# LargeWorldModel/LWM

Measured on AMD Instinct MI355X. Metric: tokens/sec fwd+bwd, LWM-7B RingAttention hot path (32 layers x 32 heads x 128), higher is better.
Workload: dtype bf16 (f32 logits/softmax/accumulate)

## Files before the change

lwm_amd/csrc/attn_bwd64.h:

```cpp
#pragma once

namespace lwm {

constexpr int kD4BK = 128;
constexpr int kD4BQ = 64;
constexpr int kD4Threads = 256;
constexpr int kD4Slots = 4;
constexpr int kD4TileBytes = kD4BQ * kRowBytes;
constexpr int kD4SlotBytes = 2 * kD4TileBytes;
constexpr int kD4OffStat = kD4Slots * kD4SlotBytes;
constexpr int kD4StatBytes = 3 * kD4BQ * 4;
constexpr int kD4LdsBytes = kD4OffStat + kD4Slots * kD4StatBytes;
#ifndef LWM_D4_AHEAD
#define LWM_D4_AHEAD 6
#endif
constexpr int kD4Ahead = LWM_D4_AHEAD;
static_assert(kD4Ahead >= 1 && kD4Ahead <= 7, "prefetch distance in fragments");
static_assert((kD4Ahead % 2) == 0, "paired requests need an even distance");

struct D4Ctx {
    uint32_t qa[8];
    uint32_t tlo[4], tup[4];
    uint32_t plo[4], pup[4];
    uint32_t stat;
    float c;
    int hi;
};

#ifdef LWM_EMU
LWM_DEVICE void d4_mfma_p_first(f32x16& d, bf16x8 a, bf16x8 b) { d = mfma_32x32x16(a, b, d); }
LWM_DEVICE void d4_mfma_o_first(f32x16& d, bf16x8 a, bf16x8 b) { d = mfma_32x32x16(a, b, zero_f32x16()); }
LWM_DEVICE float d4_mul(float a, float b) { return a * b; }
LWM_DEVICE void d4_dma_b32(uint32_t voff, const char* src, lds_t dst) { glds_load_b32(src + voff, dst); }
LWM_DEVICE void d4_settle_t(f32x16&) {}
LWM_DEVICE void d4_settle_acc(f32x16 (&)[4], f32x16 (&)[4]) {}
LWM_DEVICE void d4_settle_acc4(f32x16 (&)[4]) {}
#else
LWM_DEVICE void d4_mfma_p_first(f32x16& d, bf16x8 a, bf16x8 b) {
    asm volatile("s_nop 1\n\tv_mfma_f32_32x32x16_bf16 %0, %1, %2, %0" : "+v"(d) : "v"(a), "a"(b));
}
LWM_DEVICE void d4_mfma_o_first(f32x16& d, bf16x8 a, bf16x8 b) {
    asm volatile("v_mfma_f32_32x32x16_bf16 %0, %1, %2, 0" : "=&a"(d) : "v"(a), "v"(b));
}
LWM_DEVICE float d4_mul(float a, float b) {
    float y;
    asm volatile("v_mul_f32 %0, %1, %2" : "=v"(y) : "v"(a), "v"(b));
    return y;
}
LWM_DEVICE void d4_dma_b32(uint32_t voff, const char* src, lds_t dst) {
    const uint64_t a = (uint64_t)src;
    const uint64_t u = ((uint64_t)(uint32_t)__builtin_amdgcn_readfirstlane((int)(a >> 32)) << 32) |
                       (uint32_t)__builtin_amdgcn_readfirstlane((int)a);
    asm volatile("s_mov_b32 m0, %2\n\ts_nop 0\n\tglobal_load_lds_dword %0, %1" ::"v"(voff), "s"(u), "s"(dst) : "memory");
}
LWM_DEVICE void d4_settle_t(f32x16& s) { asm volatile("s_nop 7\n\ts_nop 7" : "+v"(s)); }
LWM_DEVICE void d4_settle_acc(f32x16 (&a)[4], f32x16 (&b)[4]) {
    asm volatile("s_nop 7\n\ts_nop 7"
                 : "+a"(a[0]), "+a"(a[1]), "+a"(a[2]), "+a"(a[3]), "+a"(b[0]), "+a"(b[1]), "+a"(b[2]), "+a"(b[3]));
}
LWM_DEVICE void d4_settle_acc4(f32x16 (&a)[4]) { asm volatile("s_nop 7\n\ts_nop 7" : "+a"(a[0]), "+a"(a[1]), "+a"(a[2]), "+a"(a[3])); }
#endif

LWM_DEVICE void d4_stage_offsets(const AttnParams& p, int wave, int lane, int st, uint32_t (&vq)[4], uint32_t (&vdo)[4]) {
    const int slot = lane & 15;
    for (int j = 0; j < 4; ++j) {
        const int row = 4 * (wave + 4 * j) + (lane >> 4);
        int qrow = st * kD4BQ + row;
        qrow = qrow < p.Sq ? qrow : p.Sq - 1;
        const int rel = qrow - st * kD4BQ;
        const int col = (slot ^ swz(row)) << 3;
        vq[j] = (uint32_t)(((int64_t)rel * p.q_ss + col) * 2);
        vdo[j] = (uint32_t)(((int64_t)rel * p.do_ss + col) * 2);
    }
}

template <int HALF>
LWM_DEVICE bf16x8 d4_frag(const D4Ctx& cx, int f) {
    if (f >= 32) {
        const int g = f - 32;
        return lds_read_b128(cx.qa[g >> 1] + (g & 1) * kD4TileBytes + (HALF == 0 ? 32 * kRowBytes : 0));
    }
    if (f < 16) return lds_read_b128(cx.qa[f >> 1] + (f & 1) * kD4TileBytes + HALF * 32 * kRowBytes);
    const int j = f - 16, t = (j >> 3) & 1, db = (j >> 1) & 3;
    const uint32_t alo = HALF == 0 ? cx.plo[db] : cx.tlo[db];
    const uint32_t aup = HALF == 0 ? cx.pup[db] : cx.tup[db];
    const uint32_t off = ((j & 1) ? 0 : kD4TileBytes) + (HALF == 0 ? 32 * kRowBytes : 0) + 16 * t * kRowBytes;
    bf16x4 lo = lds_read_tr16(alo + off);
    bf16x4 up = lds_read_tr16(aup + off);
    bf16x8 o;
    o[0] = lo[0]; o[1] = lo[1]; o[2] = lo[2]; o[3] = lo[3];
    o[4] = up[0]; o[5] = up[1]; o[6] = up[2]; o[7] = up[3];
    return o;
}

struct D4Sched {
    int F[16], E[16], M[16], P[8], D[8];
};
constexpr bool d4_sched_ok(const D4Sched& c) {
    for (int e = 0; e < 16; ++e) {
        if (c.F[e] < 1 || c.F[e] > 15) return false;
        if (c.E[e] <= c.F[e] || c.M[e] <= c.E[e] || c.M[e] > 29) return false;
    }
    for (int i = 0; i < 8; ++i) {
        const int lo = i < 4 ? 8 : 16;
        if (c.P[i] < lo || c.P[i] > 29 || c.P[i] <= c.E[2 * i] || c.P[i] <= c.E[2 * i + 1]) return false;
        if (c.D[i] < lo || c.D[i] > 29 || c.D[i] <= c.M[2 * i] || c.D[i] <= c.M[2 * i + 1]) return false;
    }
    return true;
}
constexpr D4Sched kD4Sched = {
     {1, 1, 2, 2, 3, 3, 4, 4, 5, 5, 6, 6, 7, 7, 8, 8},
     {2, 3, 4, 4, 5, 6, 7, 7, 8, 9, 9, 10, 10, 11, 11, 12},
     {16, 16, 17, 17, 18, 18, 19, 19, 20, 20, 21, 21, 22, 22, 23, 23},
     {16, 17, 18, 19, 20, 21, 22, 23},
     {24, 25, 26, 27, 28, 29, 29, 29}};
static_assert(d4_sched_ok(kD4Sched), "filler schedule violates a dependency");

struct D4Dma {
    const char* q_src;
    const char* do_src;
    lds_t dst;
};

struct D4Regs {
    f32x16 s;
    f32x16 dp[2];
    float nl[16];
    float t[16];
    float ds[16];
    bf16x8 pb[2], dsb[2];
    uint32_t pw[8], dw[8];
    bf16x8 fr[8];
};

template <int G>
LWM_DEVICE void d4_fillers(const D4Ctx& cx, D4Regs& rg, const f32x16& dpu) {
#pragma unroll
    for (int e = 0; e < 16; ++e) {
        if (kD4Sched.F[e] == G) rg.t[e] = f4_fma(rg.s[e], cx.c, rg.nl[e]);
        if (kD4Sched.E[e] == G) rg.t[e] = f4_exp2(rg.t[e]);
        if (kD4Sched.M[e] == G) rg.ds[e] = d4_mul(rg.t[e], dpu[e]);
    }
#pragma unroll
    for (int i = 0; i < 8; ++i) {
        if (kD4Sched.P[i] == G) rg.pw[i] = f4_cvt_pk(rg.t[2 * i], rg.t[2 * i + 1]);
        if (kD4Sched.D[i] == G) rg.dw[i] = f4_cvt_pk(rg.ds[2 * i], rg.ds[2 * i + 1]);
    }
#pragma unroll
    for (int h = 0; h < 2; ++h) {
        int lp = 0, ld = 0;
        for (int i = 4 * h; i < 4 * h + 4; ++i) {
            lp = kD4Sched.P[i] > lp ? kD4Sched.P[i] : lp;
            ld = kD4Sched.D[i] > ld ? kD4Sched.D[i] : ld;
        }
        if (lp == G) rg.pb[h] = __builtin_bit_cast(bf16x8, u32x4{rg.pw[4 * h], rg.pw[4 * h + 1], rg.pw[4 * h + 2], rg.pw[4 * h + 3]});
        if (ld == G) rg.dsb[h] = __builtin_bit_cast(bf16x8, u32x4{rg.dw[4 * h], rg.dw[4 * h + 1], rg.dw[4 * h + 2], rg.dw[4 * h + 3]});
    }
}
template <int G0, int N>
LWM_DEVICE void d4_fill_at(int g, const D4Ctx& cx, D4Regs& rg, const f32x16& dpu) {
    if constexpr (N > 0) {
        if (g == G0) d4_fillers<G0>(cx, rg, dpu);
        else d4_fill_at<G0 + 1, N - 1>(g, cx, rg, dpu);
    }
}

template <int HALF>
LWM_DEVICE void d4_load_ndelta(uint32_t stat, f32x16& dp, int g) {
    const f32x4 v = lds_read_f32x4(stat + kD4BQ * 4 + HALF * 32 * 4 + 8 * g * 4);
    dp[4 * g + 0] = v[0]; dp[4 * g + 1] = v[1]; dp[4 * g + 2] = v[2]; dp[4 * g + 3] = v[3];
}

template <int HALF, bool HAS_PREV, bool DMA>
LWM_DEVICE void d4_x(const D4Ctx& cx, D4Regs& rg, const bf16x8 (&kf)[8], const bf16x8 (&vf)[8], const uint32_t (&vq)[4],
                     const uint32_t (&vdo)[4], const D4Dma& dm) {
    f32x16& dpn = rg.dp[HALF];
    const f32x16& dpo = rg.dp[HALF ^ 1];
#pragma unroll
    for (int m = 0; m < 16; ++m) {
        if ((m & 1) == 0) {
            rg.fr[(m + kD4Ahead) & 7] = d4_frag<HALF>(cx, m + kD4Ahead);
            rg.fr[(m + kD4Ahead + 1) & 7] = d4_frag<HALF>(cx, m + kD4Ahead + 1);
        }
        if ((m & 3) == 2) {
            const int g = m >> 2;
            const f32x4 v = lds_read_f32x4(cx.stat + HALF * 32 * 4 + 8 * g * 4);
            rg.nl[4 * g + 0] = v[0]; rg.nl[4 * g + 1] = v[1]; rg.nl[4 * g + 2] = v[2]; rg.nl[4 * g + 3] = v[3];
        }
        sched_fence();
        {
            const int f = m ^ 1;
            if (f == 0) f4_mfma_s_first(rg.s, rg.fr[0], kf[0]);
            else if ((f & 1) == 0) f4_mfma_s(rg.s, rg.fr[f & 7], kf[f >> 1]);
            else if (f == 1) d4_mfma_p_first(dpn, rg.fr[1], vf[0]);
            else f4_mfma_s(dpn, rg.fr[f & 7], vf[f >> 1]);
        }
        if (DMA && (m & 1)) {
            const int j = m >> 2;
            if ((m & 2) == 0) f4_dma1(vq[j], dm.q_src, dm.dst + 4096 * j);
            else f4_dma1(vdo[j], dm.do_src, dm.dst + kD4TileBytes + 4096 * j);
        }
        if (HAS_PREV) d4_fill_at<16, 16>(16 + m, cx, rg, dpo);
        sched_fence();
    }
}

template <int HALF, bool HAS_META>
LWM_DEVICE void d4_mask(const D4Ctx& cx, D4Regs& rg, int rel, int32_t kseg) {
#pragma unroll
    for (int g = 0; g < 4; ++g) {
        if (HAS_META) {
            const u32x4 sg = lds_read_u32x4(cx.stat + 2 * kD4BQ * 4 + HALF * 32 * 4 + 8 * g * 4);
#pragma unroll
            for (int j = 0; j < 4; ++j) {
                const bool vis = ((int32_t)sg[j] == kseg) && (8 * g + j >= rel);
                rg.s[4 * g + j] = vis ? rg.s[4 * g + j] : -INFINITY;
            }
        } else {
#pragma unroll
            for (int j = 0; j < 4; ++j) rg.s[4 * g + j] = (8 * g + j >= rel) ? rg.s[4 * g + j] : -INFINITY;
        }
    }
}

template <int HALF, bool HAS_PREV, bool NEXT, bool INIT>
LWM_DEVICE void d4_y(const D4Ctx& cx, D4Regs& rg, f32x16 (&dk)[4], f32x16 (&dv)[4], uint32_t statn) {
#pragma unroll
    for (int j = 0; j < 16; ++j) {
        const int m = 16 + j;
        if ((j & 1) == 0 && (m + kD4Ahead < 32 || NEXT)) {
            rg.fr[(m + kD4Ahead) & 7] = d4_frag<HALF>(cx, m + kD4Ahead);
            rg.fr[(m + kD4Ahead + 1) & 7] = d4_frag<HALF>(cx, m + kD4Ahead + 1);
        }
        if (NEXT && j >= 12) d4_load_ndelta<HALF ^ 1>(statn, rg.dp[HALF ^ 1], j - 12);
        sched_fence();
        if (HAS_PREV) {
            const int jf = j ^ 1;
            if (INIT && jf < 8) {
                if ((jf & 1) == 0) d4_mfma_o_first(dv[(jf >> 1) & 3], rg.fr[(16 + jf) & 7], rg.pb[0]);
                else d4_mfma_o_first(dk[(jf >> 1) & 3], rg.fr[(16 + jf) & 7], rg.dsb[0]);
            } else {
                if ((jf & 1) == 0) f4_mfma_o(dv[(jf >> 1) & 3], rg.fr[(16 + jf) & 7], rg.pb[jf >> 3]);
                else f4_mfma_o(dk[(jf >> 1) & 3], rg.fr[(16 + jf) & 7], rg.dsb[jf >> 3]);
            }
        }
        d4_fill_at<0, 16>(j, cx, rg, rg.dp[HALF]);
        sched_fence();
    }
}

template <int PAR>
LWM_DEVICE void d4_drain(const D4Ctx& cx, D4Regs& rg, f32x16 (&dk)[4], f32x16 (&dv)[4]) {
#pragma unroll
    for (int g = 16; g < 32; ++g) d4_fill_at<16, 16>(g, cx, rg, rg.dp[PAR]);
#pragma unroll
    for (int h = 0; h < 2; ++h) {
#pragma unroll
        for (int j = 0; j < 8; ++j) rg.fr[j] = d4_frag<0>(cx, 16 + 8 * h + j);
        sched_fence();
#pragma unroll
        for (int j = 0; j < 8; ++j) {
            const int jj = 8 * h + j;
            if ((jj & 1) == 0) f4_mfma_o(dv[(jj >> 1) & 3], rg.fr[j], rg.pb[jj >> 3]);
            else f4_mfma_o(dk[(jj >> 1) & 3], rg.fr[j], rg.dsb[jj >> 3]);
        }
        sched_fence();
    }
}

LWM_DEVICE void d4_store_tiles(const AttnParams& p, lds_t tb, const f32x16 (&dk)[4], const f32x16 (&dv)[4], int b, int h,
                               int row0, int lane) {
    const int l31 = lane & 31, hi = lane >> 5, col = l31 * 4;
    const int Sk = p.Sk;
    const bool carry = p.carry_in != 0, fin = p.final_out != 0;
    const int rows = Sk - (row0 + hi);
    const int64_t acc0 = ((((int64_t)b * Sk + row0 + hi) * p.H + h) * kHeadDim + col) * 4;
    const int64_t acc_step = (int64_t)2 * p.H * kHeadDim * 4;
#pragma unroll
    for (int which = 0; which < 2; ++which) {
        if (which) wave_lds_fence();
        epi_tile_write(tb, which ? dv : dk, which ? 1.0f : p.scale, l31, hi);
        wave_lds_fence();
        char* ap = (char*)(which ? p.dv_acc : p.dk_acc) + acc0;
        const int64_t o_ss = which ? p.dv_ss : p.dk_ss;
        char* op = (char*)((which ? p.dv : p.dk) + (int64_t)b * (which ? p.dv_sb : p.dk_sb) + (int64_t)(row0 + hi) * o_ss +
                           (int64_t)h * (which ? p.dv_sh : p.dk_sh) + col);
        const int64_t out_step = 2 * o_ss * 2;
        if (fin && !carry) {
#pragma unroll
            for (int i = 0; i < 16; ++i) {
                const f32x4 x = epi_tile_read(tb, i, lane);
                if (2 * i < rows) global_store_b64(op + i * out_step, u32x2{pack_bf16x2(x[0], x[1]), pack_bf16x2(x[2], x[3])});
            }
        } else if (!fin && !carry) {
#pragma unroll
            for (int i = 0; i < 16; ++i) {
                const f32x4 x = epi_tile_read(tb, i, lane);
                if (2 * i < rows) global_store_f32x4((float*)(ap + i * acc_step), x);
            }
        } else {
#pragma unroll
            for (int i = 0; i < 16; ++i) {
                f32x4 x = epi_tile_read(tb, i, lane);
                if (2 * i < rows) {
                    const f32x4 c = global_load_f32x4((const float*)(ap + i * acc_step));
                    x[0] += c[0]; x[1] += c[1]; x[2] += c[2]; x[3] += c[3];
                    if (fin) global_store_b64(op + i * out_step, u32x2{pack_bf16x2(x[0], x[1]), pack_bf16x2(x[2], x[3])});
                    else global_store_f32x4((float*)(ap + i * acc_step), x);
                }
            }
        }
    }
}

template <bool HAS_META>
LWM_DEVICE void attn_bwd_dkdv4_body(const AttnParams& p) {
#ifdef LWM_PROF
    const unsigned long long d4_entry = __builtin_amdgcn_s_memtime();
    unsigned long long d4_head = 0, d4_epi = 0;
#endif
    const lds_t lds = dyn_lds();
    const int tid = thread_idx();
    const int wave = wave_uniform(tid >> 6), lane = tid & 63, l31 = lane & 31, hi = lane >> 5;

    const int nkb = (p.Sk + kD4BK - 1) / kD4BK;
    const int HB = p.H * p.B;
    int lin = block_idx_x(), kbi, hb;
    if ((HB & 7) == 0) {
        int xcd = lin & 7, i = lin >> 3;
        hb = xcd + 8 * (i / nkb);
        kbi = i % nkb;
    } else {
        hb = lin / nkb;
        kbi = lin % nkb;
    }
    const int b = hb / p.H, h = hb % p.H;
    const bf16_t* qb = p.q + (int64_t)b * p.q_sb + (int64_t)h * p.q_sh;
    const bf16_t* kb = p.k + (int64_t)b * p.k_sb + (int64_t)h * p.k_sh;
    const bf16_t* vb = p.v + (int64_t)b * p.v_sb + (int64_t)h * p.v_sh;
    const bf16_t* dob = p.dout + (int64_t)b * p.do_sb + (int64_t)h * p.do_sh;

    const int k_row = kbi * kD4BK + wave * 32 + l31;
    const bool k_ok = k_row < p.Sk;
    const int kr = k_ok ? k_row : p.Sk - 1;
    bf16x8 kf[8], vf[8];
    for (int s = 0; s < 8; ++s) kf[s] = f4_load_agpr(kb + (int64_t)kr * p.k_ss + 16 * s + 8 * hi);
    for (int s = 0; s < 8; ++s) vf[s] = f4_load_agpr(vb + (int64_t)kr * p.v_ss + 16 * s + 8 * hi);
    const PosMap qm = q_map(p);
    const PosTab qt_ = load_postab(qm);
    const int64_t k_base = pos_base(load_postab(k_map(p)), kbi * kD4BK);
    const int64_t k_pos = k_base + k_row;
    int32_t kseg = 0;
    if (HAS_META) {
        kseg = kSegInvalid;
        if (k_ok) {
            const bool valid = p.key_valid ? (p.key_valid[(int64_t)b * p.Sk + k_row] != 0) : true;
            if (valid) kseg = p.seg_k ? p.seg_k[(int64_t)b * p.Sk + k_row] : 0;
        }
    }

    int nst = (p.Sq + kD4BQ - 1) / kD4BQ;
    int st0 = 0;
    if (p.causal) st0 = tiles_below(qt_, kD4BQ, nst, k_base + (int64_t)kbi * kD4BK - 1);
    if (HAS_META && p.segb_q && p.segb_k && st0 < nst) {
        const int nbq = (p.Sq + 31) >> 5, nbk = (p.Sk + 31) >> 5;
        int smin, smax, lo, hi2;
        seg_own_range(p.segb_k + (int64_t)b * nbk * 2, nbk, kbi * (kD4BK / 32), kD4BK / 32, smin, smax);
        seg_narrow<kD4Threads>(p.segb_q + (int64_t)b * nbq * 2, nbq, kD4BQ / 32, st0, nst, smin, smax, lds + kD4OffStat, tid, lo, hi2);
        st0 = lo;
        nst = hi2;
    }
    const int n = nst > st0 ? nst - st0 : 0;

    f32x16 dk[4], dv[4];
    if (n == 0)
        for (int i = 0; i < 4; ++i) {
            dk[i] = zero_f32x16();
            dv[i] = zero_f32x16();
        }
    if (n == 0) {
        f4_load_agpr_wait8(kf);
        f4_load_agpr_wait8(vf);
    }

    if (n > 0) {
        D4Ctx cx;
        cx.hi = hi;
        cx.c = p.scale * kLog2e;
        for (int s = 0; s < 8; ++s) cx.qa[s] = lds + tile_off(l31, 2 * s + hi);
        {
            const TrFragAddr t = frag_tr_addr(lds, lane);
            for (int db = 0; db < 4; ++db) {
                cx.tlo[db] = t.lo[db];
                cx.tup[db] = t.up[db];
                cx.plo[db] = t.lo[db];
                cx.pup[db] = t.up[db];
            }
        }
        cx.stat = lds + kD4OffStat + 16 * hi;

        const int64_t q_step_bytes = (int64_t)kD4BQ * p.q_ss * 2, do_step_bytes = (int64_t)kD4BQ * p.do_ss * 2;
        uint32_t vq[4], vdo[4];
        d4_stage_offsets(p, wave, lane, 0, vq, vdo);
        const int64_t Sqp = bwd_stat_pad(p.Sq);
        const char* stat_src = (const char*)(p.delta + bwd_stat_row((int64_t)b * p.H + h, Sqp) + (wave == 1 ? Sqp : 0));
        bool stat_on = wave < 2;
        if (HAS_META && wave == 2 && p.seg_q) {
            stat_src = (const char*)(p.seg_q + (int64_t)b * p.Sq);
            stat_on = true;
        }
        const lds_t stat_dst = lds + kD4OffStat + (uint32_t)(wave < 3 ? wave : 0) * kD4BQ * 4;
        const uint32_t vstat = (uint32_t)lane * 4;
        if (HAS_META && !p.seg_q)
            for (int sl = 0; sl < kD4Slots; ++sl)
                if (tid < kD4BQ) lds_write_i32(lds + kD4OffStat + sl * kD4StatBytes + 2 * kD4BQ * 4 + tid * 4, 0);
        auto stage_step = [&](int i) {
            const int st = nst - 1 - i;
            const lds_t dst = lds + (i & 3) * kD4SlotBytes + (uint32_t)wave * 1024;
            const char* qs = (const char*)qb + st * q_step_bytes;
            const char* ds = (const char*)dob + st * do_step_bytes;
            if (stat_on) {
                int row = st * kD4BQ + lane;
                if (HAS_META && wave == 2) row = row < p.Sq ? row : p.Sq - 1;
                glds_load_b32(stat_src + (int64_t)row * 4, stat_dst + (i & 3) * kD4StatBytes);
            }
            if (st * kD4BQ + kD4BQ > p.Sq) {
                uint32_t v2[4], d2[4];
                d4_stage_offsets(p, wave, lane, st, v2, d2);
                f4_dma<4>(v2, qs, dst);
                f4_dma<4>(d2, ds, dst + kD4TileBytes);
            } else {
                f4_dma<4>(vq, qs, dst);
                f4_dma<4>(vdo, ds, dst + kD4TileBytes);
            }
        };

        stage_step(0);
        if (n > 1) stage_step(1);
        f4_load_agpr_wait8(kf);
        f4_load_agpr_wait8(vf);
        block_sync();

        auto clamp32 = [](int64_t x) -> int { return x > (1 << 30) ? (1 << 30) : (x < -(1 << 30) ? -(1 << 30) : (int)x); };
        const int k_rel = clamp32(k_pos - p.q_start) - 4 * hi;
        PosCursor qc = cursor_begin(qt_);
        auto q_rel_of = [&](int ub) -> int {
            cursor_seek(qm, qc, ub);
            return clamp32(qc.base + ub - p.q_start);
        };
        const int mask_end = p.causal ? 32 * tiles_reaching(qt_, 32, (p.Sq + 31) / 32, k_base + (int64_t)kbi * kD4BK + wave * 32 + 31 - 1) : 0;
        auto needs_causal = [&](int ub) -> bool { return ub < mask_end; };
        const int32_t own_seg = wave_uniform(kseg);
        const bool own_uniform = HAS_META && !wave_any(kseg != own_seg || kseg == kSegInvalid);
        auto rel_of = [&](int ub) -> int {
            if (!p.causal) return -64;
            const int64_t d = (int64_t)k_rel - q_rel_of(ub);
            return d > 64 ? 64 : (d < -64 ? -64 : (int)d);
        };

        D4Regs rg;
        rg.s = zero_f32x16();
        rg.dp[0] = zero_f32x16();
        rg.dp[1] = zero_f32x16();
        for (int r = 0; r < 16; ++r) {
            rg.nl[r] = 0.0f;
            rg.t[r] = 0.0f;
            rg.ds[r] = 0.0f;
        }
        for (int t = 0; t < 2; ++t) {
            rg.pb[t] = zero_bf16x8();
            rg.dsb[t] = zero_bf16x8();
        }
        for (int j = 0; j < 8; ++j) rg.fr[j] = zero_bf16x8();
        D4Dma dm = {};
        for (int j = 0; j < kD4Ahead; ++j) rg.fr[j] = d4_frag<0>(cx, j);
        for (int g = 0; g < 4; ++g) d4_load_ndelta<0>(cx.stat, rg.dp[0], g);

#define LWM_D4_MASK(HALF_, HAS_PREV_, ub_)                                                                          \
    do {                                                                                                            \
         \
         \
        if (!(HAS_PREV_)) d4_settle_t(rg.s);            \
        if ((HAS_META && !uni_) || needs_causal(ub_)) {                                                             \
            if (HAS_PREV_) d4_settle_t(rg.s);                                                                       \
            if (HAS_META && !uni_) d4_mask<HALF_, HAS_META>(cx, rg, rel_of(ub_), kseg);                             \
            else d4_mask<HALF_, false>(cx, rg, rel_of(ub_), kseg);                                                  \
        }                                                                                                           \
    } while (0)
#ifdef LWM_PROF
        unsigned long long d4p[12] = {0, 0, 0, 0, 0, 0, 0, 0, 0, 0, 0, 0}, d4t = __builtin_amdgcn_s_memtime();
        const unsigned long long d4t0 = d4t;
        d4_head = d4t - d4_entry;
#define D4_LAP(slot)                                                  \
    do {                                                              \
        const unsigned long long now_ = __builtin_amdgcn_s_memtime(); \
        d4p[slot] += now_ - d4t;                                      \
        d4t = now_;                                                   \
    } while (0)
#if LWM_PROF > 1
#define D4_LAP2(slot) D4_LAP(slot)
#else
#define D4_LAP2(slot)
#endif
#else
#define D4_LAP(slot)
#define D4_LAP2(slot)
#endif
        int ub = (nst - 1) * kD4BQ;
        const char* q_src2 = (const char*)qb + (int64_t)(nst - 3) * q_step_bytes;
        const char* do_src2 = (const char*)dob + (int64_t)(nst - 3) * do_step_bytes;
        const char* st_src2 = stat_src + (int64_t)(nst - 3) * kD4BQ * 4;
#define LWM_D4_STEP(i, FIRST, PIPE)                                                                                 \
    do {                                                                                                            \
        if (PIPE) {                                                                                                 \
            if (stat_on) d4_dma_b32(vstat, st_src2, stat_dst + (((i) + 2) & 3) * kD4StatBytes);        \
            dm.q_src = q_src2;                                                                                      \
            dm.do_src = do_src2;                                                                                    \
            dm.dst = lds + (((i) + 2) & 3) * kD4SlotBytes + (uint32_t)wave * 1024;                                  \
            q_src2 -= q_step_bytes;                                                                                 \
            do_src2 -= do_step_bytes;                                                                               \
            st_src2 -= kD4BQ * 4;                                                                                   \
        }                                                                                                           \
        const uint32_t d_ = (((i) & 3) == 3) ? (uint32_t)(-3 * kD4SlotBytes) : (uint32_t)kD4SlotBytes;             \
        const uint32_t e_ = (((i) & 3) == 3) ? (uint32_t)(-3 * kD4StatBytes) : (uint32_t)kD4StatBytes;             \
        const int32_t segw_ = HAS_META ? seg_step_word(cx.stat - 16 * hi + 2 * kD4BQ * 4, lane) : 0;                \
        d4_x<0, !(FIRST), PIPE>(cx, rg, kf, vf, vq, vdo, dm);                                                       \
        const bool uni_ = HAS_META && seg_step_uniform(segw_, own_uniform, own_seg);                                \
        D4_LAP2(0);                                                                                                 \
        LWM_D4_MASK(0, !(FIRST), ub);                                                                               \
        D4_LAP2(1);                                                                                                 \
        d4_y<0, !(FIRST), true, false>(cx, rg, dk, dv, cx.stat);                                                           \
        D4_LAP2(2);                                                                                                 \
        d4_x<1, true, false>(cx, rg, kf, vf, vq, vdo, dm);                                                           \
        for (int s_ = 0; s_ < 8; ++s_) cx.qa[s_] += d_;                                                             \
        D4_LAP2(3);                                                                                                 \
        LWM_D4_MASK(1, true, ub + 32);                                                                              \
        D4_LAP2(4);                                                                                                 \
        d4_y<1, true, true, FIRST>(cx, rg, dk, dv, cx.stat + e_);                                                          \
        D4_LAP(5);                                                                                                  \
        ub -= kD4BQ;                                                                                                \
          \
          \
        if ((FIRST) || !(PIPE)) d4_settle_acc(dk, dv);                                                              \
        glds_wait_all();                                                                                            \
        D4_LAP(6);                                                                                                  \
        block_sync_lds();                                                                                           \
        D4_LAP(7);                                                                                                  \
        for (int db_ = 0; db_ < 4; ++db_) {                                                                         \
            cx.plo[db_] = cx.tlo[db_];                                                                              \
            cx.pup[db_] = cx.tup[db_];                                                                              \
            cx.tlo[db_] += d_;                                                                                      \
            cx.tup[db_] += d_;                                                                                      \
        }                                                                                                           \
        cx.stat += e_;                                                                                              \
        D4_LAP(8);                                                                                                  \
    } while (0)

        int i = 0;
        if (n > 2) {
            LWM_D4_STEP(0, true, true);
#ifdef LWM_PROF
            for (int j = 0; j < 12; ++j) d4p[j] = 0;
            d4t = __builtin_amdgcn_s_memtime();
#endif
            for (i = 1; i + 2 < n; ++i) {
                LWM_D4_STEP(i, false, true);
#ifdef LWM_PROF
                d4p[9] += 1;
#endif
            }
#ifdef LWM_PROF
            if (!HAS_META && hb == 0 && kbi == 0 && lane == 0 && p.out_acc) {
                d4p[10] = __builtin_amdgcn_s_memtime() - d4t0;
                for (int j = 0; j < 11; ++j) ((unsigned long long*)p.out_acc)[wave * 16 + j] = d4p[j];
            }
#endif
            for (; i < n; ++i) LWM_D4_STEP(i, false, false);
        } else {
            LWM_D4_STEP(0, true, false);
            if (n > 1) LWM_D4_STEP(1, false, false);
        }
#undef LWM_D4_STEP
#undef D4_LAP
#undef D4_LAP2
#undef LWM_D4_MASK
        d4_drain<1>(cx, rg, dk, dv);
        d4_settle_acc(dk, dv);
    }

    d4_settle_acc(dk, dv);
#ifdef LWM_PROF
    d4_epi = __builtin_amdgcn_s_memtime() - d4_entry;
#endif
    block_sync_lds();
    d4_store_tiles(p, lds + (uint32_t)wave * kEpiTileBytes, dk, dv, b, h, kbi * kD4BK + wave * 32, lane);
#ifdef LWM_PROF
    if (!HAS_META && hb == 0 && kbi == 0 && lane == 0 && p.out_acc) {
        asm volatile("s_waitcnt vmcnt(0)" ::: "memory");
        unsigned long long* o_ = (unsigned long long*)p.out_acc + wave * 16;
        o_[11] = __builtin_amdgcn_s_memtime() - d4_entry;
        o_[12] = d4_head;
        o_[13] = d4_epi;
    }
#endif
}


LWM_KERNEL(kD4Threads) void attn_bwd_dkdv4_kernel(AttnParams p) { attn_bwd_dkdv4_body<false>(p); }
LWM_KERNEL(kD4Threads) void attn_bwd_dkdv4_meta_kernel(AttnParams p) { attn_bwd_dkdv4_body<true>(p); }


constexpr int kQ4BQ = 128;
constexpr int kQ4BK = 64;
constexpr int kQ4OffMeta = kD4Slots * kD4SlotBytes;
constexpr int kQ4LdsBytes = kQ4OffMeta + kD4Slots * kQ4BK * 4;

LWM_DEVICE int q4_swz(int row) {
    const int r = row & 15;
    return (((r & 7) << 1) | (r >> 3)) ^ ((r >= 4 && r < 12) ? 1 : 0);
}
LWM_DEVICE uint32_t q4_tile_off(int row, int slot) { return (uint32_t)(row * kRowBytes + ((slot ^ q4_swz(row)) << 4)); }

struct Q4Sched {
    int F[16], E[16], M[16], D[8];
};
constexpr bool q4_sched_ok(const Q4Sched& c) {
    int load[48] = {};
    for (int e = 0; e < 16; ++e) {
        if (c.F[e] < 3 || c.E[e] <= c.F[e] || c.M[e] <= c.E[e] || c.M[e] > 45) return false;
        load[c.F[e]] += 1;
        load[c.E[e]] += 2;
        load[c.M[e]] += 1;
    }
    for (int i = 0; i < 8; ++i) {
        if (c.D[i] < 16 || c.D[i] > 45 || c.D[i] <= c.M[2 * i] || c.D[i] <= c.M[2 * i + 1]) return false;
        load[c.D[i]] += 1;
    }
    for (int g = 0; g < 48; ++g)
        if (load[g] > 2) return false;
    return true;
}
constexpr Q4Sched kQ4Sched = {
     {3, 4, 5, 6, 7, 8, 9, 10, 11, 12, 13, 13, 14, 14, 15, 15},
     {16, 17, 18, 19, 20, 21, 22, 23, 24, 25, 26, 27, 28, 29, 30, 31},
     {32, 32, 33, 33, 34, 34, 35, 35, 36, 36, 37, 37, 38, 38, 39, 39},
     {40, 40, 41, 41, 42, 42, 43, 43}};
static_assert(q4_sched_ok(kQ4Sched), "filler schedule violates a dependency or the issue budget of a gap");

struct Q4Ctx {
    uint32_t ka[4];
    uint32_t tlo[8];
    uint32_t plo[8];
    uint32_t meta;
    float c, nl[2];
};

struct Q4Regs {
    f32x4 s[2][4], dp[2][4];
    f32x4 ndl[2];
    float t[16], ds[16];
    bf16x8 dsb[2];
    uint32_t dw[8];
    bf16x8 fr[8];
};

#ifdef LWM_EMU
LWM_DEVICE f32x4 mfma_16x16x32(bf16x8 a, bf16x8 b, f32x4 c) {
    emu::Wave& w = emu::g_blk->waves[emu::g_lane->tid >> 6];
    const int l = emu::g_lane->tid & 63;
    w.a[l] = a;
    w.b[l] = b;
    emu::wave_sync();
    f32x4 d;
    const int col = l & 15, g = l >> 4;
    for (int j = 0; j < 4; ++j) {
        const int row = 4 * g + j;
        float s = c[j];
        for (int k = 0; k < 32; ++k) s += (float)w.a[(k >> 3) * 16 + row][k & 7] * (float)w.b[(k >> 3) * 16 + col][k & 7];
        d[j] = s;
    }
    emu::wave_sync();
    return d;
}
LWM_DEVICE void q4_mfma_first(f32x4& d, bf16x8 a, bf16x8 b) { d = mfma_16x16x32(a, b, f32x4{0.0f, 0.0f, 0.0f, 0.0f}); }
LWM_DEVICE void q4_mfma(f32x4& d, bf16x8 a, bf16x8 b) { d = mfma_16x16x32(a, b, d); }
LWM_DEVICE void q4_mfma_c_first(f32x4& d, bf16x8 a, bf16x8 b, const f32x4& c) { d = mfma_16x16x32(a, b, c); }
LWM_DEVICE void q4_mfma_o(f32x4& d, bf16x8 a, bf16x8 b) { d = mfma_16x16x32(a, b, d); }
LWM_DEVICE void q4_mfma_o_first(f32x4& d, bf16x8 a, bf16x8 b) { d = mfma_16x16x32(a, b, f32x4{0.0f, 0.0f, 0.0f, 0.0f}); }
LWM_DEVICE void q4_opaque(f32x4 (&)[2]) {}
LWM_DEVICE void q4_settle_t(f32x4 (&)[4]) {}
LWM_DEVICE void q4_settle_acc(f32x4 (&)[16]) {}
#else
LWM_DEVICE void q4_mfma_first(f32x4& d, bf16x8 a, bf16x8 b) {
    asm volatile("v_mfma_f32_16x16x32_bf16 %0, %1, %2, 0" : "=&v"(d) : "v"(a), "a"(b));
}
LWM_DEVICE void q4_mfma(f32x4& d, bf16x8 a, bf16x8 b) {
    asm volatile("v_mfma_f32_16x16x32_bf16 %0, %1, %2, %0" : "+v"(d) : "v"(a), "a"(b));
}
LWM_DEVICE void q4_mfma_c_first(f32x4& d, bf16x8 a, bf16x8 b, const f32x4& c) {
    asm volatile("s_nop 1\n\tv_mfma_f32_16x16x32_bf16 %0, %1, %2, %3" : "=&v"(d) : "v"(a), "a"(b), "v"(c));
}
LWM_DEVICE void q4_mfma_o(f32x4& d, bf16x8 a, bf16x8 b) {
    asm volatile("v_mfma_f32_16x16x32_bf16 %0, %1, %2, %0" : "+a"(d) : "v"(a), "v"(b));
}
LWM_DEVICE void q4_mfma_o_first(f32x4& d, bf16x8 a, bf16x8 b) {
    asm volatile("v_mfma_f32_16x16x32_bf16 %0, %1, %2, 0" : "=&a"(d) : "v"(a), "v"(b));
}
LWM_DEVICE void q4_opaque(f32x4 (&x)[2]) { asm volatile("" : "+v"(x[0]), "+v"(x[1])); }
LWM_DEVICE void q4_settle_t(f32x4 (&s)[4]) { asm volatile("s_nop 7\n\ts_nop 7" : "+v"(s[0]), "+v"(s[1]), "+v"(s[2]), "+v"(s[3])); }
LWM_DEVICE void q4_settle_acc(f32x4 (&a)[16]) {
    asm volatile("s_nop 7\n\ts_nop 7"
                 : "+a"(a[0]), "+a"(a[1]), "+a"(a[2]), "+a"(a[3]), "+a"(a[4]), "+a"(a[5]), "+a"(a[6]), "+a"(a[7]), "+a"(a[8]),
                   "+a"(a[9]), "+a"(a[10]), "+a"(a[11]), "+a"(a[12]), "+a"(a[13]), "+a"(a[14]), "+a"(a[15]));
}
#endif

template <int HALF>
LWM_DEVICE bf16x8 q4_frag(const Q4Ctx& cx, int f) {
    if (f >= 24) {
        const int g = f - 24;
        return lds_read_b128(cx.ka[g >> 2] + (g & 1) * kD4TileBytes + ((g >> 1) & 1) * 16 * kRowBytes + (HALF == 0 ? 32 * kRowBytes : 0));
    }
    if (f < 16) return lds_read_b128(cx.ka[f >> 2] + (f & 1) * kD4TileBytes + ((f >> 1) & 1) * 16 * kRowBytes + HALF * 32 * kRowBytes);
    const int db = f - 16;
    const uint32_t a = (HALF == 0 ? cx.plo[db] : cx.tlo[db]) + (HALF == 0 ? 32 * kRowBytes : 0);
    bf16x4 lo = lds_read_tr16(a);
    bf16x4 up = lds_read_tr16(a + 16 * kRowBytes);
    bf16x8 o;
    o[0] = lo[0]; o[1] = lo[1]; o[2] = lo[2]; o[3] = lo[3];
    o[4] = up[0]; o[5] = up[1]; o[6] = up[2]; o[7] = up[3];
    return o;
}

template <int G, int PAR>
LWM_DEVICE void q4_fillers(const Q4Ctx& cx, Q4Regs& rg) {
#pragma unroll
    for (int e = 0; e < 16; ++e) {
        if (kQ4Sched.F[e] == G) rg.t[e] = f4_fma(rg.s[PAR][e >> 2][e & 3], cx.c, cx.nl[e >> 3]);
        if (kQ4Sched.E[e] == G) rg.t[e] = f4_exp2(rg.t[e]);
        if (kQ4Sched.M[e] == G) rg.ds[e] = d4_mul(rg.t[e], rg.dp[PAR][e >> 2][e & 3]);
    }
#pragma unroll
    for (int i = 0; i < 8; ++i)
        if (kQ4Sched.D[i] == G) rg.dw[i] = f4_cvt_pk(rg.ds[2 * i], rg.ds[2 * i + 1]);
#pragma unroll
    for (int h = 0; h < 2; ++h) {
        int ld = 0;
        for (int i = 4 * h; i < 4 * h + 4; ++i) ld = kQ4Sched.D[i] > ld ? kQ4Sched.D[i] : ld;
        if (ld == G) rg.dsb[h] = __builtin_bit_cast(bf16x8, u32x4{rg.dw[4 * h], rg.dw[4 * h + 1], rg.dw[4 * h + 2], rg.dw[4 * h + 3]});
    }
}
template <int HALF, bool HAS_PREV, bool DMA, int M = 0>
LWM_DEVICE void q4_x(const Q4Ctx& cx, Q4Regs& rg, const bf16x8 (&qf)[8], const bf16x8 (&dof)[8], const uint32_t (&vk)[4],
                     const uint32_t (&vv)[4], const D4Dma& dm) {
    if constexpr (M < 32) {
        if constexpr ((M & 3) == 0) {
            constexpr int f0 = (M >> 1) + kD4Ahead;
            rg.fr[f0 & 7] = q4_frag<HALF>(cx, f0);
            sched_fence();
            rg.fr[(f0 + 1) & 7] = q4_frag<HALF>(cx, f0 + 1);
        }
        sched_fence();
        {
            constexpr int f = (M >> 1) ^ 1, qh = M & 1;
            constexpr int s = f >> 2, t = 2 * qh + ((f >> 1) & 1);
            if constexpr ((f & 1) == 0) {
                if constexpr (s == 0) q4_mfma_first(rg.s[HALF][t], rg.fr[f & 7], qf[4 * qh]);
                else q4_mfma(rg.s[HALF][t], rg.fr[f & 7], qf[4 * qh + s]);
            } else {
                if constexpr (s == 0) q4_mfma_c_first(rg.dp[HALF][t], rg.fr[f & 7], dof[4 * qh], rg.ndl[qh]);
                else q4_mfma(rg.dp[HALF][t], rg.fr[f & 7], dof[4 * qh + s]);
            }
        }
        if constexpr (DMA && (M & 3) == 3) {
            constexpr int i = M >> 2, j = i >> 1;
            if constexpr ((i & 1) == 0) f4_dma1(vk[j], dm.q_src, dm.dst + 4096 * j);
            else f4_dma1(vv[j], dm.do_src, dm.dst + kD4TileBytes + 4096 * j);
        }
        if constexpr (HAS_PREV) q4_fillers<16 + M, HALF ^ 1>(cx, rg);
        sched_fence();
        q4_x<HALF, HAS_PREV, DMA, M + 1>(cx, rg, qf, dof, vk, vv, dm);
    }
}

template <int HALF, bool HAS_META>
LWM_DEVICE void q4_mask(const Q4Ctx& cx, f32x4 (&s)[4], const int (&rel)[2], const int32_t (&seg_q)[2]) {
#pragma unroll
    for (int kh = 0; kh < 2; ++kh) {
        u32x4 sg = {0u, 0u, 0u, 0u};
        if (HAS_META) sg = lds_read_u32x4(cx.meta + HALF * 32 * 4 + 16 * kh * 4);
#pragma unroll
        for (int qh = 0; qh < 2; ++qh)
#pragma unroll
            for (int j = 0; j < 4; ++j) {
                const bool vis = (!HAS_META || (int32_t)sg[j] == seg_q[qh]) && (16 * kh + j <= rel[qh]);
                s[2 * qh + kh][j] = vis ? s[2 * qh + kh][j] : -INFINITY;
            }
    }
}

template <int HALF, bool HAS_PREV, bool INIT, int J = 0>
LWM_DEVICE void q4_y(const Q4Ctx& cx, Q4Regs& rg, f32x4 (&dq)[16]) {
    if constexpr (J < 16) {
        if constexpr ((J & 3) == 0) {
            constexpr int f0 = 16 + (J >> 1) + kD4Ahead;
            rg.fr[f0 & 7] = q4_frag<HALF>(cx, f0);
            sched_fence();
            rg.fr[(f0 + 1) & 7] = q4_frag<HALF>(cx, f0 + 1);
        }
        sched_fence();
        if constexpr (HAS_PREV) {
            constexpr int db = (J >> 1) ^ 1, qh = J & 1;
            if constexpr (INIT) q4_mfma_o_first(dq[2 * db + qh], rg.fr[(16 + db) & 7], rg.dsb[qh]);
            else q4_mfma_o(dq[2 * db + qh], rg.fr[(16 + db) & 7], rg.dsb[qh]);
        }
        q4_fillers<J, HALF>(cx, rg);
        sched_fence();
        q4_y<HALF, HAS_PREV, INIT, J + 1>(cx, rg, dq);
    }
}

template <int PAR, int G = 16>
LWM_DEVICE void q4_drain_fill(const Q4Ctx& cx, Q4Regs& rg) {
    if constexpr (G < 48) {
        q4_fillers<G, PAR>(cx, rg);
        q4_drain_fill<PAR, G + 1>(cx, rg);
    }
}
template <int J = 0>
LWM_DEVICE void q4_drain_mfma(Q4Regs& rg, f32x4 (&dq)[16]) {
    if constexpr (J < 16) {
        q4_mfma_o(dq[J], rg.fr[J >> 1], rg.dsb[J & 1]);
        q4_drain_mfma<J + 1>(rg, dq);
    }
}
template <int PAR>
LWM_DEVICE void q4_drain(const Q4Ctx& cx, Q4Regs& rg, f32x4 (&dq)[16]) {
    q4_drain_fill<PAR>(cx, rg);
#pragma unroll
    for (int j = 0; j < 8; ++j) rg.fr[j] = q4_frag<0>(cx, 16 + j);
    sched_fence();
    q4_drain_mfma(rg, dq);
}

LWM_DEVICE void q4_stage_offsets(const AttnParams& p, int wave, int lane, int st, uint32_t (&vk)[4], uint32_t (&vv)[4]) {
    const int slot = lane & 15;
    for (int j = 0; j < 4; ++j) {
        const int row = 4 * (wave + 4 * j) + (lane >> 4);
        int krow = st * kQ4BK + row;
        krow = krow < p.Sk ? krow : p.Sk - 1;
        const int rel = krow - st * kQ4BK;
        const int col = (slot ^ q4_swz(row)) << 3;
        vk[j] = (uint32_t)(((int64_t)rel * p.k_ss + col) * 2);
        vv[j] = (uint32_t)(((int64_t)rel * p.v_ss + col) * 2);
    }
}

template <int QH>
LWM_DEVICE void q4_store(const AttnParams& p, const f32x4 (&dq)[16], int b, int h, int q_row, int g4) {
    const bool carry = p.carry_in != 0, fin = p.final_out != 0;
    const float sc = p.scale;
    bf16_t* const op = p.dq + (int64_t)b * p.dq_sb + (int64_t)q_row * p.dq_ss + (int64_t)h * p.dq_sh + 4 * g4;
    float* const ap = p.dq_acc + (int64_t)b * p.dqa_sb + (int64_t)q_row * p.dqa_ss + (int64_t)h * p.dqa_sh + 4 * g4;
    if (fin && !carry) {
#pragma unroll
        for (int db = 0; db < 8; ++db) {
            const f32x4 a = dq[2 * db + QH];
            global_store_b64(op + 16 * db, u32x2{pack_bf16x2(a[0] * sc, a[1] * sc), pack_bf16x2(a[2] * sc, a[3] * sc)});
        }
    } else {
#pragma unroll
        for (int db = 0; db < 8; ++db) {
            const f32x4 a = dq[2 * db + QH];
            float o0 = a[0] * sc, o1 = a[1] * sc, o2 = a[2] * sc, o3 = a[3] * sc;
            if (carry) {
                const f32x4 c = global_load_f32x4(ap + 16 * db);
                o0 += c[0]; o1 += c[1]; o2 += c[2]; o3 += c[3];
            }
            if (fin) global_store_b64(op + 16 * db, u32x2{pack_bf16x2(o0, o1), pack_bf16x2(o2, o3)});
            else global_store_f32x4(ap + 16 * db, f32x4{o0, o1, o2, o3});
        }
    }
}

template <bool HAS_META>
LWM_DEVICE void attn_bwd_dq4_body(const AttnParams& p) {
    const lds_t lds = dyn_lds();
    const int tid = thread_idx();
    const int wave = wave_uniform(tid >> 6), lane = tid & 63, l15 = lane & 15, g4 = lane >> 4;

    const int nqb = (p.Sq + kQ4BQ - 1) / kQ4BQ;
    const int HB = p.H * p.B;
    int lin = block_idx_x(), qbi, hb;
    if ((HB & 7) == 0) {
        int xcd = lin & 7, i = lin >> 3;
        hb = xcd + 8 * (i / nqb);
        qbi = nqb - 1 - (i % nqb);
    } else {
        hb = lin / nqb;
        qbi = nqb - 1 - (lin % nqb);
    }
    const int b = hb / p.H, h = hb % p.H;
    const bf16_t* qb = p.q + (int64_t)b * p.q_sb + (int64_t)h * p.q_sh;
    const bf16_t* kb = p.k + (int64_t)b * p.k_sb + (int64_t)h * p.k_sh;
    const bf16_t* vb = p.v + (int64_t)b * p.v_sb + (int64_t)h * p.v_sh;
    const bf16_t* dob = p.dout + (int64_t)b * p.do_sb + (int64_t)h * p.do_sh;

    int q_row[2], qr[2];
    bool q_ok[2];
#pragma unroll
    for (int qh = 0; qh < 2; ++qh) {
        q_row[qh] = qbi * kQ4BQ + wave * 32 + 16 * qh + l15;
        q_ok[qh] = q_row[qh] < p.Sq;
        qr[qh] = q_ok[qh] ? q_row[qh] : p.Sq - 1;
    }
    bf16x8 qf[8], dof[8];
#pragma unroll
    for (int i = 0; i < 8; ++i) qf[i] = f4_load_agpr(qb + (int64_t)qr[i >> 2] * p.q_ss + 32 * (i & 3) + 8 * g4);
#pragma unroll
    for (int i = 0; i < 8; ++i) dof[i] = f4_load_agpr(dob + (int64_t)qr[i >> 2] * p.do_ss + 32 * (i & 3) + 8 * g4);
    Q4Ctx cx;
    Q4Regs rg;
    {
        const int64_t Sqp = bwd_stat_pad(p.Sq), srow = bwd_stat_row((int64_t)b * p.H + h, Sqp);
#pragma unroll
        for (int qh = 0; qh < 2; ++qh) {
            cx.nl[qh] = q_ok[qh] ? p.delta[srow + qr[qh]] : -INFINITY;
            const float nd = p.delta[srow + Sqp + qr[qh]];
#pragma unroll
            for (int r = 0; r < 4; ++r) rg.ndl[qh][r] = nd;
        }
        q4_opaque(rg.ndl);
    }
    cx.c = p.scale * kLog2e;
    int32_t seg_q[2];
#pragma unroll
    for (int qh = 0; qh < 2; ++qh) seg_q[qh] = (HAS_META && q_ok[qh] && p.seg_q) ? p.seg_q[(int64_t)b * p.Sq + q_row[qh]] : 0;
    const PosMap km = k_map(p);
    const PosTab kt_ = load_postab(km);
    const int64_t q_base = pos_base(load_postab(q_map(p)), qbi * kQ4BQ);

    const int nst_all = (p.Sk + kQ4BK - 1) / kQ4BK;
    int nst = nst_all, st0 = 0;
    const int q_last = (qbi * kQ4BQ + kQ4BQ < p.Sq ? qbi * kQ4BQ + kQ4BQ : p.Sq) - 1;
    if (p.causal) nst = tiles_reaching(kt_, kQ4BK, nst_all, q_base + q_last);
    if (HAS_META && p.segb_q && p.segb_k && nst > 0) {
        const int nbq = (p.Sq + 31) >> 5, nbk = (p.Sk + 31) >> 5;
        int smin, smax, lo, hi2;
        seg_own_range(p.segb_q + (int64_t)b * nbq * 2, nbq, qbi * (kQ4BQ / 32), kQ4BQ / 32, smin, smax);
        seg_narrow<kD4Threads>(p.segb_k + (int64_t)b * nbk * 2, nbk, kQ4BK / 32, 0, nst, smin, smax, lds + kQ4OffMeta, tid, lo, hi2);
        st0 = lo;
        nst = hi2;
    }
    const int n = nst > st0 ? nst - st0 : 0;

    f32x4 dq[16];
    if (n == 0)
#pragma unroll
        for (int i = 0; i < 16; ++i) dq[i] = f32x4{0.0f, 0.0f, 0.0f, 0.0f};
    if (n == 0) {
        f4_load_agpr_wait8(qf);
        f4_load_agpr_wait8(dof);
    }

    if (n > 0) {
#pragma unroll
        for (int s = 0; s < 4; ++s) cx.ka[s] = lds + q4_tile_off(l15, 4 * s + g4);
#pragma unroll
        for (int db = 0; db < 8; ++db) {
            cx.tlo[db] = lds + q4_tile_off(4 * g4 + (l15 >> 2), 2 * db + ((l15 & 3) >> 1)) + (l15 & 1) * 8;
            cx.plo[db] = cx.tlo[db];
        }
        cx.meta = lds + kQ4OffMeta + 16 * g4;
        const int64_t k_step_bytes = (int64_t)kQ4BK * p.k_ss * 2, v_step_bytes = (int64_t)kQ4BK * p.v_ss * 2;
        uint32_t vk[4], vv[4];
        q4_stage_offsets(p, wave, lane, 0, vk, vv);
        auto meta_stage = [&](int i) {
            if (HAS_META && tid < kQ4BK) {
                const int krow = (st0 + i) * kQ4BK + tid;
                const int kr = krow < p.Sk ? krow : p.Sk - 1;
                const uint8_t kvalid = p.key_valid ? p.key_valid[(int64_t)b * p.Sk + kr] : (uint8_t)1;
                const int32_t kseg = p.seg_k ? p.seg_k[(int64_t)b * p.Sk + kr] : 0;
                lds_write_i32(lds + kQ4OffMeta + (i & 3) * kQ4BK * 4 + tid * 4, (krow < p.Sk && kvalid != 0) ? kseg : kSegInvalid);
            }
        };
        auto stage_step = [&](int i) {
            const int st = st0 + i;
            const lds_t dst = lds + (i & 3) * kD4SlotBytes + (uint32_t)wave * 1024;
            const char* ks = (const char*)kb + st * k_step_bytes;
            const char* vs = (const char*)vb + st * v_step_bytes;
            if (st * kQ4BK + kQ4BK > p.Sk) {
                uint32_t v2[4], d2[4];
                q4_stage_offsets(p, wave, lane, st, v2, d2);
                f4_dma<4>(v2, ks, dst);
                f4_dma<4>(d2, vs, dst + kD4TileBytes);
            } else {
                f4_dma<4>(vk, ks, dst);
                f4_dma<4>(vv, vs, dst + kD4TileBytes);
            }
            meta_stage(i);
        };
        const bool ragged = (p.Sk % kQ4BK) != 0;
        const int n_pipe_end = (ragged && nst == nst_all) ? n - 1 : n;

        stage_step(0);
        if (n > 1) stage_step(1);
        f4_load_agpr_wait8(qf);
        f4_load_agpr_wait8(dof);
        block_sync();

        auto clamp32 = [](int64_t x) -> int { return x > (1 << 30) ? (1 << 30) : (x < -(1 << 30) ? -(1 << 30) : (int)x); };
        int q_rel[2];
#pragma unroll
        for (int qh = 0; qh < 2; ++qh) q_rel[qh] = clamp32(q_base + q_row[qh] - p.k_start) - 4 * g4;
        PosCursor kc = cursor_begin(kt_);
        auto k_rel_of = [&](int ub) -> int {
            cursor_seek(km, kc, ub);
            return clamp32(kc.base + ub - p.k_start);
        };
        const int mask_from = p.causal ? 32 * tiles_below(kt_, 32, (p.Sk + 31) / 32, q_base + (int64_t)qbi * kQ4BQ + wave * 32) : 0x7fffffff;
        auto needs_causal = [&](int ub) -> bool { return ub >= mask_from; };
        const int32_t own_seg = wave_uniform(seg_q[0]);
        const bool own_uniform = HAS_META && !wave_any((q_ok[0] && seg_q[0] != own_seg) || (q_ok[1] && seg_q[1] != own_seg));
        auto rel_of = [&](int ub, int (&rel)[2]) {
            if (!p.causal) {
                rel[0] = rel[1] = 64;
                return;
            }
            const int kr = k_rel_of(ub);
#pragma unroll
            for (int qh = 0; qh < 2; ++qh) {
                const int64_t d = (int64_t)q_rel[qh] - kr;
                rel[qh] = d > 64 ? 64 : (d < -64 ? -64 : (int)d);
            }
        };

#pragma unroll
        for (int par = 0; par < 2; ++par)
#pragma unroll
            for (int t = 0; t < 4; ++t) {
                rg.s[par][t] = f32x4{0.0f, 0.0f, 0.0f, 0.0f};
                rg.dp[par][t] = f32x4{0.0f, 0.0f, 0.0f, 0.0f};
            }
#pragma unroll
        for (int r = 0; r < 16; ++r) {
            rg.t[r] = 0.0f;
            rg.ds[r] = 0.0f;
        }
#pragma unroll
        for (int t = 0; t < 2; ++t) rg.dsb[t] = zero_bf16x8();
#pragma unroll
        for (int j = 0; j < 8; ++j) rg.fr[j] = zero_bf16x8();
        D4Dma dm = {};
#pragma unroll
        for (int j = 0; j < kD4Ahead; ++j) rg.fr[j] = q4_frag<0>(cx, j);

#define LWM_Q4_MASK(HALF_, HAS_PREV_, ub_)                                                                          \
    do {                                                                                                            \
        if (!(HAS_PREV_)) q4_settle_t(rg.s[HALF_]);      \
        if ((HAS_META && !uni_) || needs_causal(ub_)) {                                                             \
            if (HAS_PREV_) q4_settle_t(rg.s[HALF_]);                                                                \
            int rel_[2];                                                                                            \
            rel_of(ub_, rel_);                                                                                      \
            if (HAS_META && !uni_) q4_mask<HALF_, HAS_META>(cx, rg.s[HALF_], rel_, seg_q);                          \
            else q4_mask<HALF_, false>(cx, rg.s[HALF_], rel_, seg_q);                                               \
        }                                                                                                           \
    } while (0)
        int ub = st0 * kQ4BK;
        const char* k_src2 = (const char*)kb + (int64_t)(st0 + 2) * k_step_bytes;
        const char* v_src2 = (const char*)vb + (int64_t)(st0 + 2) * v_step_bytes;
#define LWM_Q4_STEP(i, FIRST, PIPE)                                                                                 \
    do {                                                                                                            \
        if (PIPE) {                                                                                                 \
            dm.q_src = k_src2;                                                                                      \
            dm.do_src = v_src2;                                                                                     \
            dm.dst = lds + (((i) + 2) & 3) * kD4SlotBytes + (uint32_t)wave * 1024;                                  \
            k_src2 += k_step_bytes;                                                                                 \
            v_src2 += v_step_bytes;                                                                                 \
            meta_stage((i) + 2);                                                                                    \
        }                                                                                                           \
        const uint32_t d_ = (((i) & 3) == 3) ? (uint32_t)(-3 * kD4SlotBytes) : (uint32_t)kD4SlotBytes;             \
        const uint32_t e_ = (((i) & 3) == 3) ? (uint32_t)(-3 * kQ4BK * 4) : (uint32_t)(kQ4BK * 4);                 \
        const int32_t segw_ = HAS_META ? seg_step_word(cx.meta - 16 * g4, lane) : 0;                               \
        q4_x<0, !(FIRST), PIPE>(cx, rg, qf, dof, vk, vv, dm);                                                       \
        const bool uni_ = HAS_META && seg_step_uniform(segw_, own_uniform, own_seg);                                \
        LWM_Q4_MASK(0, !(FIRST), ub);                                                                               \
        q4_y<0, !(FIRST), false>(cx, rg, dq);                                                                       \
        q4_x<1, true, false>(cx, rg, qf, dof, vk, vv, dm);                                                          \
        for (int s_ = 0; s_ < 4; ++s_) cx.ka[s_] += d_;                                                             \
        LWM_Q4_MASK(1, true, ub + 32);                                                                              \
        q4_y<1, true, FIRST>(cx, rg, dq);                                                                           \
        ub += kQ4BK;                                                                                                \
        if ((FIRST) || !(PIPE)) q4_settle_acc(dq);                                                                  \
        glds_wait_all();                                                                                            \
        block_sync_lds();                                                                                           \
        for (int db_ = 0; db_ < 8; ++db_) {                                                                         \
            cx.plo[db_] = cx.tlo[db_];                                                                              \
            cx.tlo[db_] += d_;                                                                                      \
        }                                                                                                           \
        cx.meta += e_;                                                                                              \
    } while (0)

        int i = 0;
        if (n_pipe_end > 2) {
            LWM_Q4_STEP(0, true, true);
            for (i = 1; i + 2 < n_pipe_end; ++i) LWM_Q4_STEP(i, false, true);
            if (n_pipe_end < n) {
                stage_step(n - 1);
                glds_wait_all();
                block_sync_lds();
            }
            for (; i < n; ++i) LWM_Q4_STEP(i, false, false);
        } else {
            if (n > 2) {
                stage_step(2);
                glds_wait_all();
                block_sync_lds();
            }
            LWM_Q4_STEP(0, true, false);
            for (i = 1; i < n; ++i) LWM_Q4_STEP(i, false, false);
        }
#undef LWM_Q4_STEP
#undef LWM_Q4_MASK
        q4_drain<1>(cx, rg, dq);
        q4_settle_acc(dq);
    }

    q4_settle_acc(dq);
    if (q_ok[0]) q4_store<0>(p, dq, b, h, q_row[0], g4);
    if (q_ok[1]) q4_store<1>(p, dq, b, h, q_row[1], g4);
}

LWM_KERNEL(kD4Threads) void attn_bwd_dq4_kernel(AttnParams p) { attn_bwd_dq4_body<false>(p); }
LWM_KERNEL(kD4Threads) void attn_bwd_dq4_meta_kernel(AttnParams p) { attn_bwd_dq4_body<true>(p); }

}
```

Baseline: 30990.

## Switch dK/dV backward kernel from 32x32 to 16x16 MFMA tiles

Rewrites the D4 backward kernel's inner loops to use v_mfma_f32_16x16x32 instead of 32x32x16. Score and dP accumulators are split into 2x2 f32x4 quadrants, dK/dV into 16 f32x4 tiles each, and the swizzle moves to the q4 layout. The loops become compile-time recursive templates with a filler schedule spread over 64 issue gaps and capped at two filler ops per gap. The delta term is now folded into the first dP MFMA as the C operand. The aim is finer interleaving of softmax/exp fillers with MFMA issue and shorter dependency latency, at the cost of more MFMA instructions and different register pressure.

```diff
diff --git a/lwm_amd/csrc/attn_bwd64.h b/lwm_amd/csrc/attn_bwd64.h
--- a/lwm_amd/csrc/attn_bwd64.h
+++ b/lwm_amd/csrc/attn_bwd64.h
@@ -18,29 +18,64 @@
 static_assert(kD4Ahead >= 1 && kD4Ahead <= 7, "prefetch distance in fragments");
 static_assert((kD4Ahead % 2) == 0, "paired requests need an even distance");
 
-struct D4Ctx {
-    uint32_t qa[8];
-    uint32_t tlo[4], tup[4];
-    uint32_t plo[4], pup[4];
-    uint32_t stat;
-    float c;
-    int hi;
-};
+LWM_DEVICE int q4_swz(int row) {
+    const int r = row & 15;
+    return (((r & 7) << 1) | (r >> 3)) ^ ((r >= 4 && r < 12) ? 1 : 0);
+}
+LWM_DEVICE uint32_t q4_tile_off(int row, int slot) { return (uint32_t)(row * kRowBytes + ((slot ^ q4_swz(row)) << 4)); }
 
 #ifdef LWM_EMU
-LWM_DEVICE void d4_mfma_p_first(f32x16& d, bf16x8 a, bf16x8 b) { d = mfma_32x32x16(a, b, d); }
-LWM_DEVICE void d4_mfma_o_first(f32x16& d, bf16x8 a, bf16x8 b) { d = mfma_32x32x16(a, b, zero_f32x16()); }
+LWM_DEVICE f32x4 mfma_16x16x32(bf16x8 a, bf16x8 b, f32x4 c) {
+    emu::Wave& w = emu::g_blk->waves[emu::g_lane->tid >> 6];
+    const int l = emu::g_lane->tid & 63;
+    w.a[l] = a;
+    w.b[l] = b;
+    emu::wave_sync();
+    f32x4 d;
+    const int col = l & 15, g = l >> 4;
+    for (int j = 0; j < 4; ++j) {
+        const int row = 4 * g + j;
+        float s = c[j];
+        for (int k = 0; k < 32; ++k) s += (float)w.a[(k >> 3) * 16 + row][k & 7] * (float)w.b[(k >> 3) * 16 + col][k & 7];
+        d[j] = s;
+    }
+    emu::wave_sync();
+    return d;
+}
+LWM_DEVICE void q4_mfma_first(f32x4& d, bf16x8 a, bf16x8 b) { d = mfma_16x16x32(a, b, f32x4{0.0f, 0.0f, 0.0f, 0.0f}); }
+LWM_DEVICE void q4_mfma(f32x4& d, bf16x8 a, bf16x8 b) { d = mfma_16x16x32(a, b, d); }
+LWM_DEVICE void q4_mfma_c_first(f32x4& d, bf16x8 a, bf16x8 b, const f32x4& c) { d = mfma_16x16x32(a, b, c); }
+LWM_DEVICE void q4_mfma_o(f32x4& d, bf16x8 a, bf16x8 b) { d = mfma_16x16x32(a, b, d); }
+LWM_DEVICE void q4_mfma_o_first(f32x4& d, bf16x8 a, bf16x8 b) { d = mfma_16x16x32(a, b, f32x4{0.0f, 0.0f, 0.0f, 0.0f}); }
+LWM_DEVICE void q4_opaque(f32x4 (&)[2]) {}
+LWM_DEVICE void q4_settle_t(f32x4 (&)[4]) {}
+LWM_DEVICE void q4_settle_acc(f32x4 (&)[16]) {}
 LWM_DEVICE float d4_mul(float a, float b) { return a * b; }
 LWM_DEVICE void d4_dma_b32(uint32_t voff, const char* src, lds_t dst) { glds_load_b32(src + voff, dst); }
-LWM_DEVICE void d4_settle_t(f32x16&) {}
-LWM_DEVICE void d4_settle_acc(f32x16 (&)[4], f32x16 (&)[4]) {}
 LWM_DEVICE void d4_settle_acc4(f32x16 (&)[4]) {}
+LWM_DEVICE void d4_settle_t(f32x4 (&)[2][2]) {}
 #else
-LWM_DEVICE void d4_mfma_p_first(f32x16& d, bf16x8 a, bf16x8 b) {
-    asm volatile("s_nop 1\n\tv_mfma_f32_32x32x16_bf16 %0, %1, %2, %0" : "+v"(d) : "v"(a), "a"(b));
-}
-LWM_DEVICE void d4_mfma_o_first(f32x16& d, bf16x8 a, bf16x8 b) {
-    asm volatile("v_mfma_f32_32x32x16_bf16 %0, %1, %2, 0" : "=&a"(d) : "v"(a), "v"(b));
+LWM_DEVICE void q4_mfma_first(f32x4& d, bf16x8 a, bf16x8 b) {
+    asm volatile("v_mfma_f32_16x16x32_bf16 %0, %1, %2, 0" : "=&v"(d) : "v"(a), "a"(b));
+}
+LWM_DEVICE void q4_mfma(f32x4& d, bf16x8 a, bf16x8 b) {
+    asm volatile("v_mfma_f32_16x16x32_bf16 %0, %1, %2, %0" : "+v"(d) : "v"(a), "a"(b));
+}
+LWM_DEVICE void q4_mfma_c_first(f32x4& d, bf16x8 a, bf16x8 b, const f32x4& c) {
+    asm volatile("s_nop 1\n\tv_mfma_f32_16x16x32_bf16 %0, %1, %2, %3" : "=&v"(d) : "v"(a), "a"(b), "v"(c));
+}
+LWM_DEVICE void q4_mfma_o(f32x4& d, bf16x8 a, bf16x8 b) {
+    asm volatile("v_mfma_f32_16x16x32_bf16 %0, %1, %2, %0" : "+a"(d) : "v"(a), "v"(b));
+}
+LWM_DEVICE void q4_mfma_o_first(f32x4& d, bf16x8 a, bf16x8 b) {
+    asm volatile("v_mfma_f32_16x16x32_bf16 %0, %1, %2, 0" : "=&a"(d) : "v"(a), "v"(b));
+}
+LWM_DEVICE void q4_opaque(f32x4 (&x)[2]) { asm volatile("" : "+v"(x[0]), "+v"(x[1])); }
+LWM_DEVICE void q4_settle_t(f32x4 (&s)[4]) { asm volatile("s_nop 7\n\ts_nop 7" : "+v"(s[0]), "+v"(s[1]), "+v"(s[2]), "+v"(s[3])); }
+LWM_DEVICE void q4_settle_acc(f32x4 (&a)[16]) {
+    asm volatile("s_nop 7\n\ts_nop 7"
+                 : "+a"(a[0]), "+a"(a[1]), "+a"(a[2]), "+a"(a[3]), "+a"(a[4]), "+a"(a[5]), "+a"(a[6]), "+a"(a[7]), "+a"(a[8]),
+                   "+a"(a[9]), "+a"(a[10]), "+a"(a[11]), "+a"(a[12]), "+a"(a[13]), "+a"(a[14]), "+a"(a[15]));
 }
 LWM_DEVICE float d4_mul(float a, float b) {
     float y;
@@ -53,13 +88,21 @@
                        (uint32_t)__builtin_amdgcn_readfirstlane((int)a);
     asm volatile("s_mov_b32 m0, %2\n\ts_nop 0\n\tglobal_load_lds_dword %0, %1" ::"v"(voff), "s"(u), "s"(dst) : "memory");
 }
-LWM_DEVICE void d4_settle_t(f32x16& s) { asm volatile("s_nop 7\n\ts_nop 7" : "+v"(s)); }
-LWM_DEVICE void d4_settle_acc(f32x16 (&a)[4], f32x16 (&b)[4]) {
-    asm volatile("s_nop 7\n\ts_nop 7"
-                 : "+a"(a[0]), "+a"(a[1]), "+a"(a[2]), "+a"(a[3]), "+a"(b[0]), "+a"(b[1]), "+a"(b[2]), "+a"(b[3]));
-}
+LWM_DEVICE void d4_settle_t(f32x4 (&s)[2][2]) { asm volatile("s_nop 7\n\ts_nop 7" : "+v"(s[0][0]), "+v"(s[0][1]), "+v"(s[1][0]), "+v"(s[1][1])); }
 LWM_DEVICE void d4_settle_acc4(f32x16 (&a)[4]) { asm volatile("s_nop 7\n\ts_nop 7" : "+a"(a[0]), "+a"(a[1]), "+a"(a[2]), "+a"(a[3])); }
 #endif
+LWM_DEVICE void d4_settle_acc(f32x4 (&dk)[16], f32x4 (&dv)[16]) {
+    q4_settle_acc(dk);
+    q4_settle_acc(dv);
+}
+
+struct D4Ctx {
+    uint32_t qa[4];
+    uint32_t tlo[8];
+    uint32_t plo[8];
+    uint32_t stat;
+    float c;
+};
 
 LWM_DEVICE void d4_stage_offsets(const AttnParams& p, int wave, int lane, int st, uint32_t (&vq)[4], uint32_t (&vdo)[4]) {
     const int slot = lane & 15;
@@ -68,7 +111,7 @@
         int qrow = st * kD4BQ + row;
         qrow = qrow < p.Sq ? qrow : p.Sq - 1;
         const int rel = qrow - st * kD4BQ;
-        const int col = (slot ^ swz(row)) << 3;
+        const int col = (slot ^ q4_swz(row)) << 3;
         vq[j] = (uint32_t)(((int64_t)rel * p.q_ss + col) * 2);
         vdo[j] = (uint32_t)(((int64_t)rel * p.do_ss + col) * 2);
     }
@@ -78,15 +121,13 @@
 LWM_DEVICE bf16x8 d4_frag(const D4Ctx& cx, int f) {
     if (f >= 32) {
         const int g = f - 32;
-        return lds_read_b128(cx.qa[g >> 1] + (g & 1) * kD4TileBytes + (HALF == 0 ? 32 * kRowBytes : 0));
-    }
-    if (f < 16) return lds_read_b128(cx.qa[f >> 1] + (f & 1) * kD4TileBytes + HALF * 32 * kRowBytes);
-    const int j = f - 16, t = (j >> 3) & 1, db = (j >> 1) & 3;
-    const uint32_t alo = HALF == 0 ? cx.plo[db] : cx.tlo[db];
-    const uint32_t aup = HALF == 0 ? cx.pup[db] : cx.tup[db];
-    const uint32_t off = ((j & 1) ? 0 : kD4TileBytes) + (HALF == 0 ? 32 * kRowBytes : 0) + 16 * t * kRowBytes;
-    bf16x4 lo = lds_read_tr16(alo + off);
-    bf16x4 up = lds_read_tr16(aup + off);
+        return lds_read_b128(cx.qa[g >> 2] + (g & 1) * kD4TileBytes + ((g >> 1) & 1) * 16 * kRowBytes + (HALF == 0 ? 32 * kRowBytes : 0));
+    }
+    if (f < 16) return lds_read_b128(cx.qa[f >> 2] + (f & 1) * kD4TileBytes + ((f >> 1) & 1) * 16 * kRowBytes + HALF * 32 * kRowBytes);
+    const int j = f - 16, db = j >> 1;
+    const uint32_t a = (HALF == 0 ? cx.plo[db] : cx.tlo[db]) + ((j & 1) ? 0 : kD4TileBytes) + (HALF == 0 ? 32 * kRowBytes : 0);
+    bf16x4 lo = lds_read_tr16(a);
+    bf16x4 up = lds_read_tr16(a + 16 * kRowBytes);
     bf16x8 o;
     o[0] = lo[0]; o[1] = lo[1]; o[2] = lo[2]; o[3] = lo[3];
     o[4] = up[0]; o[5] = up[1]; o[6] = up[2]; o[7] = up[3];
@@ -97,24 +138,30 @@
     int F[16], E[16], M[16], P[8], D[8];
 };
 constexpr bool d4_sched_ok(const D4Sched& c) {
+    int load[64] = {};
     for (int e = 0; e < 16; ++e) {
-        if (c.F[e] < 1 || c.F[e] > 15) return false;
-        if (c.E[e] <= c.F[e] || c.M[e] <= c.E[e] || c.M[e] > 29) return false;
+        if (c.F[e] < 3 || c.F[e] > 31 || c.E[e] <= c.F[e] || c.M[e] <= c.E[e] || c.M[e] > 61) return false;
+        load[c.F[e]] += 1;
+        load[c.E[e]] += 2;
+        load[c.M[e]] += 1;
     }
     for (int i = 0; i < 8; ++i) {
-        const int lo = i < 4 ? 8 : 16;
-        if (c.P[i] < lo || c.P[i] > 29 || c.P[i] <= c.E[2 * i] || c.P[i] <= c.E[2 * i + 1]) return false;
-        if (c.D[i] < lo || c.D[i] > 29 || c.D[i] <= c.M[2 * i] || c.D[i] <= c.M[2 * i + 1]) return false;
-    }
+        if (c.P[i] < 32 || c.P[i] > 61 || c.P[i] <= c.E[2 * i] || c.P[i] <= c.E[2 * i + 1]) return false;
+        if (c.D[i] < 32 || c.D[i] > 61 || c.D[i] <= c.M[2 * i] || c.D[i] <= c.M[2 * i + 1]) return false;
+        load[c.P[i]] += 1;
+        load[c.D[i]] += 1;
+    }
+    for (int g = 0; g < 64; ++g)
+        if (load[g] > 2) return false;
     return true;
 }
 constexpr D4Sched kD4Sched = {
-     {1, 1, 2, 2, 3, 3, 4, 4, 5, 5, 6, 6, 7, 7, 8, 8},
-     {2, 3, 4, 4, 5, 6, 7, 7, 8, 9, 9, 10, 10, 11, 11, 12},
-     {16, 16, 17, 17, 18, 18, 19, 19, 20, 20, 21, 21, 22, 22, 23, 23},
-     {16, 17, 18, 19, 20, 21, 22, 23},
-     {24, 25, 26, 27, 28, 29, 29, 29}};
-static_assert(d4_sched_ok(kD4Sched), "filler schedule violates a dependency");
+     {3, 4, 5, 6, 7, 8, 9, 10, 11, 12, 13, 14, 15, 16, 17, 18},
+     {20, 22, 24, 26, 28, 30, 32, 33, 34, 35, 36, 37, 38, 39, 40, 41},
+     {42, 42, 43, 43, 44, 44, 45, 45, 46, 46, 47, 47, 48, 48, 49, 49},
+     {50, 50, 51, 51, 52, 52, 53, 53},
+     {54, 54, 55, 55, 56, 56, 57, 57}};
+static_assert(d4_sched_ok(kD4Sched), "filler schedule violates a dependency or the issue budget of a gap");
 
 struct D4Dma {
     const char* q_src;
@@ -123,9 +170,10 @@
 };
 
 struct D4Regs {
-    f32x16 s;
-    f32x16 dp[2];
-    float nl[16];
+    f32x4 s[2][2];
+    f32x4 dp[2][2][2];
+    f32x4 nl[2];
+    f32x4 ndl[2];
     float t[16];
     float ds[16];
     bf16x8 pb[2], dsb[2];
@@ -133,13 +181,14 @@
     bf16x8 fr[8];
 };
 
-template <int G>
-LWM_DEVICE void d4_fillers(const D4Ctx& cx, D4Regs& rg, const f32x16& dpu) {
+template <int G, int PAR>
+LWM_DEVICE void d4_fillers(const D4Ctx& cx, D4Regs& rg) {
 #pragma unroll
     for (int e = 0; e < 16; ++e) {
-        if (kD4Sched.F[e] == G) rg.t[e] = f4_fma(rg.s[e], cx.c, rg.nl[e]);
+        const int kh = e >> 3, qh = (e >> 2) & 1, j = e & 3;
+        if (kD4Sched.F[e] == G) rg.t[e] = f4_fma(rg.s[qh][kh][j], cx.c, rg.nl[qh][j]);
         if (kD4Sched.E[e] == G) rg.t[e] = f4_exp2(rg.t[e]);
-        if (kD4Sched.M[e] == G) rg.ds[e] = d4_mul(rg.t[e], dpu[e]);
+        if (kD4Sched.M[e] == G) rg.ds[e] = d4_mul(rg.t[e], rg.dp[PAR][qh][kh][j]);
     }
 #pragma unroll
     for (int i = 0; i < 8; ++i) {
@@ -157,118 +206,133 @@
         if (ld == G) rg.dsb[h] = __builtin_bit_cast(bf16x8, u32x4{rg.dw[4 * h], rg.dw[4 * h + 1], rg.dw[4 * h + 2], rg.dw[4 * h + 3]});
     }
 }
-template <int G0, int N>
-LWM_DEVICE void d4_fill_at(int g, const D4Ctx& cx, D4Regs& rg, const f32x16& dpu) {
-    if constexpr (N > 0) {
-        if (g == G0) d4_fillers<G0>(cx, rg, dpu);
-        else d4_fill_at<G0 + 1, N - 1>(g, cx, rg, dpu);
-    }
-}
-
-template <int HALF>
-LWM_DEVICE void d4_load_ndelta(uint32_t stat, f32x16& dp, int g) {
-    const f32x4 v = lds_read_f32x4(stat + kD4BQ * 4 + HALF * 32 * 4 + 8 * g * 4);
-    dp[4 * g + 0] = v[0]; dp[4 * g + 1] = v[1]; dp[4 * g + 2] = v[2]; dp[4 * g + 3] = v[3];
-}
-
-template <int HALF, bool HAS_PREV, bool DMA>
+
+template <int HALF, int QH>
+LWM_DEVICE void d4_load_ndelta(uint32_t stat, D4Regs& rg) {
+    rg.ndl[QH] = lds_read_f32x4(stat + kD4BQ * 4 + HALF * 32 * 4 + QH * 16 * 4);
+}
+
+template <int HALF, bool HAS_PREV, bool DMA, int M = 0>
 LWM_DEVICE void d4_x(const D4Ctx& cx, D4Regs& rg, const bf16x8 (&kf)[8], const bf16x8 (&vf)[8], const uint32_t (&vq)[4],
                      const uint32_t (&vdo)[4], const D4Dma& dm) {
-    f32x16& dpn = rg.dp[HALF];
-    const f32x16& dpo = rg.dp[HALF ^ 1];
-#pragma unroll
-    for (int m = 0; m < 16; ++m) {
-        if ((m & 1) == 0) {
-            rg.fr[(m + kD4Ahead) & 7] = d4_frag<HALF>(cx, m + kD4Ahead);
-            rg.fr[(m + kD4Ahead + 1) & 7] = d4_frag<HALF>(cx, m + kD4Ahead + 1);
-        }
-        if ((m & 3) == 2) {
-            const int g = m >> 2;
-            const f32x4 v = lds_read_f32x4(cx.stat + HALF * 32 * 4 + 8 * g * 4);
-            rg.nl[4 * g + 0] = v[0]; rg.nl[4 * g + 1] = v[1]; rg.nl[4 * g + 2] = v[2]; rg.nl[4 * g + 3] = v[3];
-        }
+    if constexpr (M < 32) {
+        if constexpr ((M & 3) == 0) {
+            constexpr int f0 = (M >> 1) + kD4Ahead;
+            rg.fr[f0 & 7] = d4_frag<HALF>(cx, f0);
+            sched_fence();
+            rg.fr[(f0 + 1) & 7] = d4_frag<HALF>(cx, f0 + 1);
+        }
+        if constexpr (M == 18 || M == 22) rg.nl[(M - 18) >> 2] = lds_read_f32x4(cx.stat + HALF * 32 * 4 + ((M - 18) >> 2) * 16 * 4);
         sched_fence();
         {
-            const int f = m ^ 1;
-            if (f == 0) f4_mfma_s_first(rg.s, rg.fr[0], kf[0]);
-            else if ((f & 1) == 0) f4_mfma_s(rg.s, rg.fr[f & 7], kf[f >> 1]);
-            else if (f == 1) d4_mfma_p_first(dpn, rg.fr[1], vf[0]);
-            else f4_mfma_s(dpn, rg.fr[f & 7], vf[f >> 1]);
-        }
-        if (DMA && (m & 1)) {
-            const int j = m >> 2;
-            if ((m & 2) == 0) f4_dma1(vq[j], dm.q_src, dm.dst + 4096 * j);
+            constexpr int f = (M >> 1) ^ 1, kh = M & 1;
+            constexpr int s = f >> 2, qh = (f >> 1) & 1;
+            if constexpr ((f & 1) == 0) {
+                if constexpr (s == 0) q4_mfma_first(rg.s[qh][kh], rg.fr[f & 7], kf[4 * kh]);
+                else q4_mfma(rg.s[qh][kh], rg.fr[f & 7], kf[4 * kh + s]);
+            } else {
+                if constexpr (s == 0) q4_mfma_c_first(rg.dp[HALF][qh][kh], rg.fr[f & 7], vf[4 * kh], rg.ndl[qh]);
+                else q4_mfma(rg.dp[HALF][qh][kh], rg.fr[f & 7], vf[4 * kh + s]);
+            }
+        }
+        if constexpr (DMA && (M & 3) == 3) {
+            constexpr int i = M >> 2, j = i >> 1;
+            if constexpr ((i & 1) == 0) f4_dma1(vq[j], dm.q_src, dm.dst + 4096 * j);
             else f4_dma1(vdo[j], dm.do_src, dm.dst + kD4TileBytes + 4096 * j);
         }
-        if (HAS_PREV) d4_fill_at<16, 16>(16 + m, cx, rg, dpo);
+        if constexpr (HAS_PREV) d4_fillers<32 + M, HALF ^ 1>(cx, rg);
         sched_fence();
+        d4_x<HALF, HAS_PREV, DMA, M + 1>(cx, rg, kf, vf, vq, vdo, dm);
     }
 }
 
 template <int HALF, bool HAS_META>
-LWM_DEVICE void d4_mask(const D4Ctx& cx, D4Regs& rg, int rel, int32_t kseg) {
-#pragma unroll
-    for (int g = 0; g < 4; ++g) {
-        if (HAS_META) {
-            const u32x4 sg = lds_read_u32x4(cx.stat + 2 * kD4BQ * 4 + HALF * 32 * 4 + 8 * g * 4);
+LWM_DEVICE void d4_mask(const D4Ctx& cx, f32x4 (&s)[2][2], const int (&rel)[2], const int32_t (&kseg)[2]) {
+#pragma unroll
+    for (int qh = 0; qh < 2; ++qh) {
+        u32x4 sg = {0u, 0u, 0u, 0u};
+        if (HAS_META) sg = lds_read_u32x4(cx.stat + 2 * kD4BQ * 4 + HALF * 32 * 4 + qh * 16 * 4);
+#pragma unroll
+        for (int kh = 0; kh < 2; ++kh)
 #pragma unroll
             for (int j = 0; j < 4; ++j) {
-                const bool vis = ((int32_t)sg[j] == kseg) && (8 * g + j >= rel);
-                rg.s[4 * g + j] = vis ? rg.s[4 * g + j] : -INFINITY;
-            }
-        } else {
-#pragma unroll
-            for (int j = 0; j < 4; ++j) rg.s[4 * g + j] = (8 * g + j >= rel) ? rg.s[4 * g + j] : -INFINITY;
-        }
-    }
-}
-
-template <int HALF, bool HAS_PREV, bool NEXT, bool INIT>
-LWM_DEVICE void d4_y(const D4Ctx& cx, D4Regs& rg, f32x16 (&dk)[4], f32x16 (&dv)[4], uint32_t statn) {
-#pragma unroll
-    for (int j = 0; j < 16; ++j) {
-        const int m = 16 + j;
-        if ((j & 1) == 0 && (m + kD4Ahead < 32 || NEXT)) {
-            rg.fr[(m + kD4Ahead) & 7] = d4_frag<HALF>(cx, m + kD4Ahead);
-            rg.fr[(m + kD4Ahead + 1) & 7] = d4_frag<HALF>(cx, m + kD4Ahead + 1);
-        }
-        if (NEXT && j >= 12) d4_load_ndelta<HALF ^ 1>(statn, rg.dp[HALF ^ 1], j - 12);
+                const bool vis = (!HAS_META || (int32_t)sg[j] == kseg[kh]) && (16 * qh + j >= rel[kh]);
+                s[qh][kh][j] = vis ? s[qh][kh][j] : -INFINITY;
+            }
+    }
+}
+
+template <int HALF, bool HAS_PREV, bool INIT, int J = 0>
+LWM_DEVICE void d4_y(const D4Ctx& cx, D4Regs& rg, f32x4 (&dk)[16], f32x4 (&dv)[16], uint32_t statn) {
+    if constexpr (J < 32) {
+        if constexpr ((J & 3) == 0) {
+            constexpr int f0 = 16 + (J >> 1) + kD4Ahead;
+            rg.fr[f0 & 7] = d4_frag<HALF>(cx, f0);
+            sched_fence();
+            rg.fr[(f0 + 1) & 7] = d4_frag<HALF>(cx, f0 + 1);
+        }
+        if constexpr (J == 26) d4_load_ndelta<HALF ^ 1, 0>(statn, rg);
+        if constexpr (J == 30) d4_load_ndelta<HALF ^ 1, 1>(statn, rg);
         sched_fence();
-        if (HAS_PREV) {
-            const int jf = j ^ 1;
-            if (INIT && jf < 8) {
-                if ((jf & 1) == 0) d4_mfma_o_first(dv[(jf >> 1) & 3], rg.fr[(16 + jf) & 7], rg.pb[0]);
-                else d4_mfma_o_first(dk[(jf >> 1) & 3], rg.fr[(16 + jf) & 7], rg.dsb[0]);
+        if constexpr (HAS_PREV) {
+            constexpr int f = (J >> 1) ^ 1, kh = J & 1, db = f >> 1;
+            if constexpr ((f & 1) == 0) {
+                if constexpr (INIT) q4_mfma_o_first(dv[2 * db + kh], rg.fr[f & 7], rg.pb[kh]);
+                else q4_mfma_o(dv[2 * db + kh], rg.fr[f & 7], rg.pb[kh]);
             } else {
-                if ((jf & 1) == 0) f4_mfma_o(dv[(jf >> 1) & 3], rg.fr[(16 + jf) & 7], rg.pb[jf >> 3]);
-                else f4_mfma_o(dk[(jf >> 1) & 3], rg.fr[(16 + jf) & 7], rg.dsb[jf >> 3]);
-            }
-        }
-        d4_fill_at<0, 16>(j, cx, rg, rg.dp[HALF]);
+                if constexpr (INIT) q4_mfma_o_first(dk[2 * db + kh], rg.fr[f & 7], rg.dsb[kh]);
+                else q4_mfma_o(dk[2 * db + kh], rg.fr[f & 7], rg.dsb[kh]);
+            }
+        }
+        d4_fillers<J, HALF>(cx, rg);
         sched_fence();
-    }
-}
-
+        d4_y<HALF, HAS_PREV, INIT, J + 1>(cx, rg, dk, dv, statn);
+    }
+}
+
+template <int PAR, int G = 32>
+LWM_DEVICE void d4_drain_fill(const D4Ctx& cx, D4Regs& rg) {
+    if constexpr (G < 64) {
+        d4_fillers<G, PAR>(cx, rg);
+        d4_drain_fill<PAR, G + 1>(cx, rg);
+    }
+}
+template <int H, int J = 0>
+LWM_DEVICE void d4_drain_mfma(D4Regs& rg, f32x4 (&dk)[16], f32x4 (&dv)[16]) {
+    if constexpr (J < 16) {
+        constexpr int f = 8 * H + (J >> 1), kh = J & 1, db = f >> 1;
+        if constexpr ((f & 1) == 0) q4_mfma_o(dv[2 * db + kh], rg.fr[f & 7], rg.pb[kh]);
+        else q4_mfma_o(dk[2 * db + kh], rg.fr[f & 7], rg.dsb[kh]);
+        d4_drain_mfma<H, J + 1>(rg, dk, dv);
+    }
+}
 template <int PAR>
-LWM_DEVICE void d4_drain(const D4Ctx& cx, D4Regs& rg, f32x16 (&dk)[4], f32x16 (&dv)[4]) {
-#pragma unroll
-    for (int g = 16; g < 32; ++g) d4_fill_at<16, 16>(g, cx, rg, rg.dp[PAR]);
-#pragma unroll
-    for (int h = 0; h < 2; ++h) {
-#pragma unroll
-        for (int j = 0; j < 8; ++j) rg.fr[j] = d4_frag<0>(cx, 16 + 8 * h + j);
-        sched_fence();
-#pragma unroll
-        for (int j = 0; j < 8; ++j) {
-            const int jj = 8 * h + j;
-            if ((jj & 1) == 0) f4_mfma_o(dv[(jj >> 1) & 3], rg.fr[j], rg.pb[jj >> 3]);
-            else f4_mfma_o(dk[(jj >> 1) & 3], rg.fr[j], rg.dsb[jj >> 3]);
-        }
-        sched_fence();
-    }
-}
-
-LWM_DEVICE void d4_store_tiles(const AttnParams& p, lds_t tb, const f32x16 (&dk)[4], const f32x16 (&dv)[4], int b, int h,
+LWM_DEVICE void d4_drain(const D4Ctx& cx, D4Regs& rg, f32x4 (&dk)[16], f32x4 (&dv)[16]) {
+    d4_drain_fill<PAR>(cx, rg);
+#pragma unroll
+    for (int j = 0; j < 8; ++j) rg.fr[j] = d4_frag<0>(cx, 16 + j);
+    sched_fence();
+    d4_drain_mfma<0>(rg, dk, dv);
+    sched_fence();
+#pragma unroll
+    for (int j = 0; j < 8; ++j) rg.fr[j] = d4_frag<0>(cx, 24 + j);
+    sched_fence();
+    d4_drain_mfma<1>(rg, dk, dv);
+    sched_fence();
+}
+
+LWM_DEVICE void d4_epi_tile_write(lds_t tb, const f32x4 (&acc)[16], float scale, int c, int g) {
+#pragma unroll
+    for (int db = 0; db < 8; ++db)
+#pragma unroll
+        for (int kh = 0; kh < 2; ++kh) {
+            const f32x4 a = acc[2 * db + kh];
+            lds_write_f32x4(tb + (uint32_t)((16 * kh + c) * kEpiRowBytes + (16 * db + 4 * g) * 4),
+                            f32x4{a[0] * scale, a[1] * scale, a[2] * scale, a[3] * scale});
+        }
+}
+
+LWM_DEVICE void d4_store_tiles(const AttnParams& p, lds_t tb, const f32x4 (&dk)[16], const f32x4 (&dv)[16], int b, int h,
                                int row0, int lane) {
     const int l31 = lane & 31, hi = lane >> 5, col = l31 * 4;
     const int Sk = p.Sk;
@@ -279,7 +343,7 @@
 #pragma unroll
     for (int which = 0; which < 2; ++which) {
         if (which) wave_lds_fence();
-        epi_tile_write(tb, which ? dv : dk, which ? 1.0f : p.scale, l31, hi);
+        d4_epi_tile_write(tb, which ? dv : dk, which ? 1.0f : p.scale, lane & 15, lane >> 4);
         wave_lds_fence();
         char* ap = (char*)(which ? p.dv_acc : p.dk_acc) + acc0;
         const int64_t o_ss = which ? p.dv_ss : p.dk_ss;
@@ -321,7 +385,7 @@
 #endif
     const lds_t lds = dyn_lds();
     const int tid = thread_idx();
-    const int wave = wave_uniform(tid >> 6), lane = tid & 63, l31 = lane & 31, hi = lane >> 5;
+    const int wave = wave_uniform(tid >> 6), lane = tid & 63, l15 = lane & 15, g4 = lane >> 4;
 
     const int nkb = (p.Sk + kD4BK - 1) / kD4BK;
     const int HB = p.H * p.B;
@@ -340,22 +404,31 @@
     const bf16_t* vb = p.v + (int64_t)b * p.v_sb + (int64_t)h * p.v_sh;
     const bf16_t* dob = p.dout + (int64_t)b * p.do_sb + (int64_t)h * p.do_sh;
 
-    const int k_row = kbi * kD4BK + wave * 32 + l31;
-    const bool k_ok = k_row < p.Sk;
-    const int kr = k_ok ? k_row : p.Sk - 1;
+    int k_row[2], kr[2];
+    bool k_ok[2];
+#pragma unroll
+    for (int kh = 0; kh < 2; ++kh) {
+        k_row[kh] = kbi * kD4BK + wave * 32 + 16 * kh + l15;
+        k_ok[kh] = k_row[kh] < p.Sk;
+        kr[kh] = k_ok[kh] ? k_row[kh] : p.Sk - 1;
+    }
     bf16x8 kf[8], vf[8];
-    for (int s = 0; s < 8; ++s) kf[s] = f4_load_agpr(kb + (int64_t)kr * p.k_ss + 16 * s + 8 * hi);
-    for (int s = 0; s < 8; ++s) vf[s] = f4_load_agpr(vb + (int64_t)kr * p.v_ss + 16 * s + 8 * hi);
+#pragma unroll
+    for (int i = 0; i < 8; ++i) kf[i] = f4_load_agpr(kb + (int64_t)kr[i >> 2] * p.k_ss + 32 * (i & 3) + 8 * g4);
+#pragma unroll
+    for (int i = 0; i < 8; ++i) vf[i] = f4_load_agpr(vb + (int64_t)kr[i >> 2] * p.v_ss + 32 * (i & 3) + 8 * g4);
     const PosMap qm = q_map(p);
     const PosTab qt_ = load_postab(qm);
     const int64_t k_base = pos_base(load_postab(k_map(p)), kbi * kD4BK);
-    const int64_t k_pos = k_base + k_row;
-    int32_t kseg = 0;
+    int32_t kseg[2] = {0, 0};
     if (HAS_META) {
-        kseg = kSegInvalid;
-        if (k_ok) {
-            const bool valid = p.key_valid ? (p.key_valid[(int64_t)b * p.Sk + k_row] != 0) : true;
-            if (valid) kseg = p.seg_k ? p.seg_k[(int64_t)b * p.Sk + k_row] : 0;
+#pragma unroll
+        for (int kh = 0; kh < 2; ++kh) {
+            kseg[kh] = kSegInvalid;
+            if (k_ok[kh]) {
+                const bool valid = p.key_valid ? (p.key_valid[(int64_t)b * p.Sk + k_row[kh]] != 0) : true;
+                if (valid) kseg[kh] = p.seg_k ? p.seg_k[(int64_t)b * p.Sk + k_row[kh]] : 0;
+            }
         }
     }
 
@@ -372,11 +445,12 @@
     }
     const int n = nst > st0 ? nst - st0 : 0;
 
-    f32x16 dk[4], dv[4];
+    f32x4 dk[16], dv[16];
     if (n == 0)
-        for (int i = 0; i < 4; ++i) {
-            dk[i] = zero_f32x16();
-            dv[i] = zero_f32x16();
+#pragma unroll
+        for (int i = 0; i < 16; ++i) {
+            dk[i] = f32x4{0.0f, 0.0f, 0.0f, 0.0f};
+            dv[i] = f32x4{0.0f, 0.0f, 0.0f, 0.0f};
         }
     if (n == 0) {
         f4_load_agpr_wait8(kf);
@@ -385,19 +459,15 @@
 
     if (n > 0) {
         D4Ctx cx;
-        cx.hi = hi;
         cx.c = p.scale * kLog2e;
-        for (int s = 0; s < 8; ++s) cx.qa[s] = lds + tile_off(l31, 2 * s + hi);
-        {
-            const TrFragAddr t = frag_tr_addr(lds, lane);
-            for (int db = 0; db < 4; ++db) {
-                cx.tlo[db] = t.lo[db];
-                cx.tup[db] = t.up[db];
-                cx.plo[db] = t.lo[db];
-                cx.pup[db] = t.up[db];
-            }
-        }
-        cx.stat = lds + kD4OffStat + 16 * hi;
+#pragma unroll
+        for (int s = 0; s < 4; ++s) cx.qa[s] = lds + q4_tile_off(l15, 4 * s + g4);
+#pragma unroll
+        for (int db = 0; db < 8; ++db) {
+            cx.tlo[db] = lds + q4_tile_off(4 * g4 + (l15 >> 2), 2 * db + ((l15 & 3) >> 1)) + (l15 & 1) * 8;
+            cx.plo[db] = cx.tlo[db];
+        }
+        cx.stat = lds + kD4OffStat + 16 * g4;
 
         const int64_t q_step_bytes = (int64_t)kD4BQ * p.q_ss * 2, do_step_bytes = (int64_t)kD4BQ * p.do_ss * 2;
         uint32_t vq[4], vdo[4];
@@ -442,7 +512,9 @@
         block_sync();
 
         auto clamp32 = [](int64_t x) -> int { return x > (1 << 30) ? (1 << 30) : (x < -(1 << 30) ? -(1 << 30) : (int)x); };
-        const int k_rel = clamp32(k_pos - p.q_start) - 4 * hi;
+        int k_rel[2];
+#pragma unroll
+        for (int kh = 0; kh < 2; ++kh) k_rel[kh] = clamp32(k_base + k_row[kh] - p.q_start) - 4 * g4;
         PosCursor qc = cursor_begin(qt_);
         auto q_rel_of = [&](int ub) -> int {
             cursor_seek(qm, qc, ub);
@@ -450,41 +522,61 @@
         };
         const int mask_end = p.causal ? 32 * tiles_reaching(qt_, 32, (p.Sq + 31) / 32, k_base + (int64_t)kbi * kD4BK + wave * 32 + 31 - 1) : 0;
         auto needs_causal = [&](int ub) -> bool { return ub < mask_end; };
-        const int32_t own_seg = wave_uniform(kseg);
-        const bool own_uniform = HAS_META && !wave_any(kseg != own_seg || kseg == kSegInvalid);
-        auto rel_of = [&](int ub) -> int {
-            if (!p.causal) return -64;
-            const int64_t d = (int64_t)k_rel - q_rel_of(ub);
-            return d > 64 ? 64 : (d < -64 ? -64 : (int)d);
+        const int32_t own_seg = wave_uniform(kseg[0]);
+        const bool own_uniform = HAS_META && !wave_any(kseg[0] != own_seg || kseg[1] != own_seg || own_seg == kSegInvalid);
+        auto rel_of = [&](int ub, int (&rel)[2]) {
+            if (!p.causal) {
+                rel[0] = rel[1] = -64;
+                return;
+            }
+            const int qr = q_rel_of(ub);
+#pragma unroll
+            for (int kh = 0; kh < 2; ++kh) {
+                const int64_t d = (int64_t)k_rel[kh] - qr;
+                rel[kh] = d > 64 ? 64 : (d < -64 ? -64 : (int)d);
+            }
         };
 
         D4Regs rg;
-        rg.s = zero_f32x16();
-        rg.dp[0] = zero_f32x16();
-        rg.dp[1] = zero_f32x16();
+#pragma unroll
+        for (int qh = 0; qh < 2; ++qh) {
+            rg.nl[qh] = f32x4{0.0f, 0.0f, 0.0f, 0.0f};
+#pragma unroll
+            for (int kh = 0; kh < 2; ++kh) {
+                rg.s[qh][kh] = f32x4{0.0f, 0.0f, 0.0f, 0.0f};
+                rg.dp[0][qh][kh] = f32x4{0.0f, 0.0f, 0.0f, 0.0f};
+                rg.dp[1][qh][kh] = f32x4{0.0f, 0.0f, 0.0f, 0.0f};
+            }
+        }
+#pragma unroll
         for (int r = 0; r < 16; ++r) {
-            rg.nl[r] = 0.0f;
             rg.t[r] = 0.0f;
             rg.ds[r] = 0.0f;
         }
+#pragma unroll
         for (int t = 0; t < 2; ++t) {
             rg.pb[t] = zero_bf16x8();
             rg.dsb[t] = zero_bf16x8();
         }
+#pragma unroll
         for (int j = 0; j < 8; ++j) rg.fr[j] = zero_bf16x8();
         D4Dma dm = {};
+#pragma unroll
         for (int j = 0; j < kD4Ahead; ++j) rg.fr[j] = d4_frag<0>(cx, j);
-        for (int g = 0; g < 4; ++g) d4_load_ndelta<0>(cx.stat, rg.dp[0], g);
+        d4_load_ndelta<0, 0>(cx.stat, rg);
+        d4_load_ndelta<0, 1>(cx.stat, rg);
 
 #define LWM_D4_MASK(HALF_, HAS_PREV_, ub_)                                                                          \
     do {                                                                                                            \
          \
          \
-        if (!(HAS_PREV_)) d4_settle_t(rg.s);            \
+        if (!(HAS_PREV_)) d4_settle_t(rg.s);      \
         if ((HAS_META && !uni_) || needs_causal(ub_)) {                                                             \
-            if (HAS_PREV_) d4_settle_t(rg.s);                                                                       \
-            if (HAS_META && !uni_) d4_mask<HALF_, HAS_META>(cx, rg, rel_of(ub_), kseg);                             \
-            else d4_mask<HALF_, false>(cx, rg, rel_of(ub_), kseg);                                                  \
+            if (HAS_PREV_) d4_settle_t(rg.s);                                                                \
+            int rel_[2];                                                                                            \
+            rel_of(ub_, rel_);                                                                                      \
+            if (HAS_META && !uni_) d4_mask<HALF_, HAS_META>(cx, rg.s, rel_, kseg);                                  \
+            else d4_mask<HALF_, false>(cx, rg.s, rel_, kseg);                                                       \
         }                                                                                                           \
     } while (0)
 #ifdef LWM_PROF
@@ -513,7 +605,7 @@
 #define LWM_D4_STEP(i, FIRST, PIPE)                                                                                 \
     do {                                                                                                            \
         if (PIPE) {                                                                                                 \
-            if (stat_on) d4_dma_b32(vstat, st_src2, stat_dst + (((i) + 2) & 3) * kD4StatBytes);        \
+            if (stat_on) d4_dma_b32(vstat, st_src2, stat_dst + (((i) + 2) & 3) * kD4StatBytes);                     \
             dm.q_src = q_src2;                                                                                      \
             dm.do_src = do_src2;                                                                                    \
             dm.dst = lds + (((i) + 2) & 3) * kD4SlotBytes + (uint32_t)wave * 1024;                                  \
@@ -523,20 +615,20 @@
         }                                                                                                           \
         const uint32_t d_ = (((i) & 3) == 3) ? (uint32_t)(-3 * kD4SlotBytes) : (uint32_t)kD4SlotBytes;             \
         const uint32_t e_ = (((i) & 3) == 3) ? (uint32_t)(-3 * kD4StatBytes) : (uint32_t)kD4StatBytes;             \
-        const int32_t segw_ = HAS_META ? seg_step_word(cx.stat - 16 * hi + 2 * kD4BQ * 4, lane) : 0;                \
+        const int32_t segw_ = HAS_META ? seg_step_word(cx.stat - 16 * g4 + 2 * kD4BQ * 4, lane) : 0;                \
         d4_x<0, !(FIRST), PIPE>(cx, rg, kf, vf, vq, vdo, dm);                                                       \
         const bool uni_ = HAS_META && seg_step_uniform(segw_, own_uniform, own_seg);                                \
         D4_LAP2(0);                                                                                                 \
         LWM_D4_MASK(0, !(FIRST), ub);                                                                               \
         D4_LAP2(1);                                                                                                 \
-        d4_y<0, !(FIRST), true, false>(cx, rg, dk, dv, cx.stat);                                                           \
+        d4_y<0, !(FIRST), false>(cx, rg, dk, dv, cx.stat);                                                          \
         D4_LAP2(2);                                                                                                 \
-        d4_x<1, true, false>(cx, rg, kf, vf, vq, vdo, dm);                                                           \
-        for (int s_ = 0; s_ < 8; ++s_) cx.qa[s_] += d_;                                                             \
+        d4_x<1, true, false>(cx, rg, kf, vf, vq, vdo, dm);                                                          \
+        for (int s_ = 0; s_ < 4; ++s_) cx.qa[s_] += d_;                                                             \
         D4_LAP2(3);                                                                                                 \
         LWM_D4_MASK(1, true, ub + 32);                                                                              \
         D4_LAP2(4);                                                                                                 \
-        d4_y<1, true, true, FIRST>(cx, rg, dk, dv, cx.stat + e_);                                                          \
+        d4_y<1, true, FIRST>(cx, rg, dk, dv, cx.stat + e_);                                                         \
         D4_LAP(5);                                                                                                  \
         ub -= kD4BQ;                                                                                                \
           \
@@ -546,11 +638,9 @@
         D4_LAP(6);                                                                                                  \
         block_sync_lds();                                                                                           \
         D4_LAP(7);                                                                                                  \
-        for (int db_ = 0; db_ < 4; ++db_) {                                                                         \
+        for (int db_ = 0; db_ < 8; ++db_) {                                                                         \
             cx.plo[db_] = cx.tlo[db_];                                                                              \
-            cx.pup[db_] = cx.tup[db_];                                                                              \
             cx.tlo[db_] += d_;                                                                                      \
-            cx.tup[db_] += d_;                                                                                      \
         }                                                                                                           \
         cx.stat += e_;                                                                                              \
         D4_LAP(8);                                                                                                  \
@@ -615,12 +705,6 @@
 constexpr int kQ4OffMeta = kD4Slots * kD4SlotBytes;
 constexpr int kQ4LdsBytes = kQ4OffMeta + kD4Slots * kQ4BK * 4;
 
-LWM_DEVICE int q4_swz(int row) {
-    const int r = row & 15;
-    return (((r & 7) << 1) | (r >> 3)) ^ ((r >= 4 && r < 12) ? 1 : 0);
-}
-LWM_DEVICE uint32_t q4_tile_off(int row, int slot) { return (uint32_t)(row * kRowBytes + ((slot ^ q4_swz(row)) << 4)); }
-
 struct Q4Sched {
     int F[16], E[16], M[16], D[8];
 };
@@ -663,57 +747,6 @@
     uint32_t dw[8];
     bf16x8 fr[8];
 };
-
-#ifdef LWM_EMU
-LWM_DEVICE f32x4 mfma_16x16x32(bf16x8 a, bf16x8 b, f32x4 c) {
-    emu::Wave& w = emu::g_blk->waves[emu::g_lane->tid >> 6];
-    const int l = emu::g_lane->tid & 63;
-    w.a[l] = a;
-    w.b[l] = b;
-    emu::wave_sync();
-    f32x4 d;
-    const int col = l & 15, g = l >> 4;
-    for (int j = 0; j < 4; ++j) {
-        const int row = 4 * g + j;
-        float s = c[j];
-        for (int k = 0; k < 32; ++k) s += (float)w.a[(k >> 3) * 16 + row][k & 7] * (float)w.b[(k >> 3) * 16 + col][k & 7];
-        d[j] = s;
-    }
-    emu::wave_sync();
-    return d;
-}
-LWM_DEVICE void q4_mfma_first(f32x4& d, bf16x8 a, bf16x8 b) { d = mfma_16x16x32(a, b, f32x4{0.0f, 0.0f, 0.0f, 0.0f}); }
-LWM_DEVICE void q4_mfma(f32x4& d, bf16x8 a, bf16x8 b) { d = mfma_16x16x32(a, b, d); }
-LWM_DEVICE void q4_mfma_c_first(f32x4& d, bf16x8 a, bf16x8 b, const f32x4& c) { d = mfma_16x16x32(a, b, c); }
-LWM_DEVICE void q4_mfma_o(f32x4& d, bf16x8 a, bf16x8 b) { d = mfma_16x16x32(a, b, d); }
-LWM_DEVICE void q4_mfma_o_first(f32x4& d, bf16x8 a, bf16x8 b) { d = mfma_16x16x32(a, b, f32x4{0.0f, 0.0f, 0.0f, 0.0f}); }
-LWM_DEVICE void q4_opaque(f32x4 (&)[2]) {}
-LWM_DEVICE void q4_settle_t(f32x4 (&)[4]) {}
-LWM_DEVICE void q4_settle_acc(f32x4 (&)[16]) {}
-#else
-LWM_DEVICE void q4_mfma_first(f32x4& d, bf16x8 a, bf16x8 b) {
-    asm volatile("v_mfma_f32_16x16x32_bf16 %0, %1, %2, 0" : "=&v"(d) : "v"(a), "a"(b));
-}
-LWM_DEVICE void q4_mfma(f32x4& d, bf16x8 a, bf16x8 b) {
-    asm volatile("v_mfma_f32_16x16x32_bf16 %0, %1, %2, %0" : "+v"(d) : "v"(a), "a"(b));
-}
-LWM_DEVICE void q4_mfma_c_first(f32x4& d, bf16x8 a, bf16x8 b, const f32x4& c) {
-    asm volatile("s_nop 1\n\tv_mfma_f32_16x16x32_bf16 %0, %1, %2, %3" : "=&v"(d) : "v"(a), "a"(b), "v"(c));
-}
-LWM_DEVICE void q4_mfma_o(f32x4& d, bf16x8 a, bf16x8 b) {
-    asm volatile("v_mfma_f32_16x16x32_bf16 %0, %1, %2, %0" : "+a"(d) : "v"(a), "v"(b));
-}
-LWM_DEVICE void q4_mfma_o_first(f32x4& d, bf16x8 a, bf16x8 b) {
-    asm volatile("v_mfma_f32_16x16x32_bf16 %0, %1, %2, 0" : "=&a"(d) : "v"(a), "v"(b));
-}
-LWM_DEVICE void q4_opaque(f32x4 (&x)[2]) { asm volatile("" : "+v"(x[0]), "+v"(x[1])); }
-LWM_DEVICE void q4_settle_t(f32x4 (&s)[4]) { asm volatile("s_nop 7\n\ts_nop 7" : "+v"(s[0]), "+v"(s[1]), "+v"(s[2]), "+v"(s[3])); }
-LWM_DEVICE void q4_settle_acc(f32x4 (&a)[16]) {
-    asm volatile("s_nop 7\n\ts_nop 7"
-                 : "+a"(a[0]), "+a"(a[1]), "+a"(a[2]), "+a"(a[3]), "+a"(a[4]), "+a"(a[5]), "+a"(a[6]), "+a"(a[7]), "+a"(a[8]),
-                   "+a"(a[9]), "+a"(a[10]), "+a"(a[11]), "+a"(a[12]), "+a"(a[13]), "+a"(a[14]), "+a"(a[15]));
-}
-#endif
 
 template <int HALF>
 LWM_DEVICE bf16x8 q4_frag(const Q4Ctx& cx, int f) {
```

New measurement: 31240 (median of 6 runs). Within noise of the previous version (+0.8%).
